# rubengooj/pl-svo

Measured on AMD Instinct MI355X. Metric: sparse-align+pose-opt frames/sec, 640×480, ~200 pts+80 lines; 1/2/4/8 GPU, higher is better.
Workload: dtype f64

## Files before the change

include/plsvo_hip.h:

```cpp
#ifndef PLSVO_HIP_H_
#define PLSVO_HIP_H_

#include <stddef.h>
#include <stdint.h>

#ifdef __cplusplus
extern "C" {
#endif

#define PLSVO_MAX_LEVELS 8
#define PLSVO_PATCH_SIZE 4
#define PLSVO_PATCH_AREA 16

#define PLSVO_OK              0
#define PLSVO_E_INVALID      -1
#define PLSVO_E_NODEVICE     -2
#define PLSVO_E_HIP          -3
#define PLSVO_E_CAPACITY     -4
#define PLSVO_E_STATE        -5
#define PLSVO_E_RCCL         -6

typedef struct plsvo_ctx plsvo_ctx;

typedef struct plsvo_pinhole {
  double fx, fy, cx, cy;
  int32_t width, height;
} plsvo_pinhole;


int plsvo_hip_create(int device_id, void* stream, plsvo_ctx** out);
int plsvo_hip_create_on_stream(int device_id, void* stream, plsvo_ctx** out);
void plsvo_hip_destroy(plsvo_ctx* ctx);
#define PLSVO_OPT_LDLT_FLAVOUR 1
#define PLSVO_OPT_ALIGN_THREADS 2
#define PLSVO_OPT_POSEOPT_THREADS 3
#define PLSVO_OPT_ALIGN_REORDER 4
#define PLSVO_OPT_POSEOPT_REORDER 5
#define PLSVO_OPT_ALIGN_TAIL_SPLIT 6
#define PLSVO_OPT_POSEOPT_REFILL 7
int plsvo_hip_set_option(plsvo_ctx* ctx, int option, int value);
const char* plsvo_hip_last_error(const plsvo_ctx* ctx);
void* plsvo_hip_stream(plsvo_ctx* ctx);
int plsvo_hip_synchronize(plsvo_ctx* ctx);


int plsvo_hip_config_pyramids(plsvo_ctx* ctx, int n_slots, int width, int height, int n_levels);

int plsvo_hip_upload_pyramid(plsvo_ctx* ctx, int slot, int n_levels,
                             const uint8_t* const* level_ptr, const int* width, const int* height,
                             const int* stride_bytes);

int plsvo_hip_build_pyramid(plsvo_ctx* ctx, int slot, const uint8_t* level0, int stride_bytes,
                            int rounding);
int plsvo_hip_build_pyramids_dev(plsvo_ctx* ctx, int first_slot, int n, const void* d_level0,
                                 int stride_bytes, size_t image_pitch_bytes, int rounding);
int plsvo_hip_copy_slots(plsvo_ctx* ctx, int dst_first, int src_first, int n);
int plsvo_hip_download_level(plsvo_ctx* ctx, int slot, int level, uint8_t* out);


typedef struct plsvo_pinhole_radtan {
  plsvo_pinhole cam;
  double d[5];
} plsvo_pinhole_radtan;

#define PLSVO_MAX_RECTIFY_MAPS 8

int plsvo_rectify_map(const plsvo_pinhole_radtan* cam, int16_t* xy, uint16_t* frac);
int plsvo_hip_config_rectify(plsvo_ctx* ctx, const plsvo_pinhole_radtan* cam, int flip_vertical, int* map_id);
int plsvo_hip_rectify_build_pyramid(plsvo_ctx* ctx, int map_id, int slot, const uint8_t* raw, int stride_bytes, int rounding);
int plsvo_hip_rectify_build_pyramids_dev(plsvo_ctx* ctx, int map_id, int first_slot, int n, const void* d_raw,
                                         int stride_bytes, size_t image_pitch_bytes, int rounding);


typedef struct plsvo_corner { int32_t x, y; float score; int32_t level; } plsvo_corner;

typedef struct plsvo_detect_params {
  int32_t cell_size;
  int32_t n_levels;
  int32_t fast_threshold;
  int32_t reserved0;
  double  detection_threshold;
} plsvo_detect_params;

int plsvo_detect_grid(int width, int height, int cell_size, int* cols, int* rows);
int plsvo_detect_cell(int cols, int cell_size, double px_x, double px_y);
int plsvo_hip_detect_fast(plsvo_ctx* ctx, int first_slot, int n, const plsvo_detect_params* params, const uint8_t* occupancy,
                          plsvo_corner* corners, int32_t* counts);
int plsvo_hip_detect_fast_dev(plsvo_ctx* ctx, int first_slot, int n, const plsvo_detect_params* params, const uint8_t* d_occupancy,
                              plsvo_corner* d_corners, int32_t* d_counts);
int plsvo_hip_detect_stages(plsvo_ctx* ctx, int slot, int level, int fast_threshold, uint8_t* score, uint8_t* survives);


typedef struct plsvo_align_in {
  int32_t ref_slot, cur_slot;
  plsvo_pinhole cam;
  int32_t max_level, min_level;
  int32_t n_iter;
  int32_t reserved0;
  double eps;
  double T_cur_from_ref[7];
  int32_t n_pts, n_seg;
  const double* pt_px;
  const double* pt_xyz_ref;
  const double* seg_spx;
  const double* seg_epx;
  const double* seg_len;
  const double* seg_p_ref;
  const double* seg_q_ref;
  const uint8_t* seg_alive_in;
} plsvo_align_in;

typedef struct plsvo_align_out {
  double T_cur_from_ref[7];
  uint64_t n_meas;
  uint64_t n_tracked;
  double H[36];
  double chi2;
  uint8_t* seg_alive_out;
  int32_t iters_per_level[PLSVO_MAX_LEVELS];
  int32_t status;
  int32_t reserved0;
} plsvo_align_out;
// ... 4 lines not shown
  int32_t stop;
  uint64_t n_meas;
  double new_chi2;
  double H[36], Jres[6], x[6];
  double T_after[7];
} plsvo_align_iterlog;

int plsvo_sparse_align(plsvo_ctx* ctx, const plsvo_align_in* in, plsvo_align_out* out);
int plsvo_sparse_align_batch(plsvo_ctx* ctx, int n, const plsvo_align_in* in, plsvo_align_out* out);

int plsvo_align_stage(plsvo_ctx* ctx, int n, const plsvo_align_in* in);
int plsvo_align_run(plsvo_ctx* ctx);
int plsvo_align_fetch(plsvo_ctx* ctx, int n, plsvo_align_out* out);

int plsvo_align_slot_layout(const plsvo_align_in* in, int level, int32_t* seg_code, int32_t* n_slots, int32_t* long_lines,
                            long long* n_patches);

int plsvo_align_set_trace(plsvo_ctx* ctx, int max_records_per_job);
int plsvo_align_fetch_trace(plsvo_ctx* ctx, int job, plsvo_align_iterlog* out, int max_records,
                            int* n_records);

const double* plsvo_align_poses_dev(plsvo_ctx* ctx);
int plsvo_align_copy_poses(plsvo_ctx* ctx, double* d_dst);

int plsvo_align_work(plsvo_ctx* ctx, uint64_t* patch_levels, uint64_t* patch_iters);
int plsvo_align_launch_order(plsvo_ctx* ctx, int n, int32_t* order);
int plsvo_align_tail_frames(plsvo_ctx* ctx, int* tail_frames);
int plsvo_align_work_points(plsvo_ctx* ctx, uint64_t* point_patch_iters);

int plsvo_align_chi2_ties(plsvo_ctx* ctx, uint64_t* iterations, uint64_t* ties, uint64_t* near_ties_without_terms);


typedef struct plsvo_poseopt_in {
  double T_f_w[7];
  double fx;
  double reproj_thresh;
  int32_t n_iter;
  int32_t n_iter_ref;
  int32_t n_pts, n_seg;
  const double* pt_f;
  const double* pt_pos;
  const int32_t* pt_level;
  const double* seg_line;
  const double* seg_spos;
  const double* seg_epos;
  const int32_t* seg_level;
} plsvo_poseopt_in;

typedef struct plsvo_poseopt_out {
  double T_f_w[7];
  double cov[36];
  double estimated_scale, error_init, error_final;
  uint64_t num_obs_pt, num_obs_ls;
  uint8_t* pt_keep;
  uint8_t* seg_keep;
  int32_t iters;
  int32_t iters_ref;
  int32_t status;
  int32_t reserved0;
} plsvo_poseopt_out;

typedef struct plsvo_poseopt_iterlog {
  int32_t phase;
  int32_t iter;
  int32_t accepted;
  int32_t reserved0;
  double new_chi2;
  double A[36], b[6], dT[6];
  double T_after[7];
} plsvo_poseopt_iterlog;

int plsvo_pose_optimize(plsvo_ctx* ctx, const plsvo_poseopt_in* in, plsvo_poseopt_out* out);
int plsvo_pose_optimize_batch(plsvo_ctx* ctx, int n, const plsvo_poseopt_in* in, plsvo_poseopt_out* out);
int plsvo_poseopt_stage(plsvo_ctx* ctx, int n, const plsvo_poseopt_in* in);
int plsvo_poseopt_run(plsvo_ctx* ctx);
int plsvo_poseopt_fetch(plsvo_ctx* ctx, int n, plsvo_poseopt_out* out);
int plsvo_poseopt_set_trace(plsvo_ctx* ctx, int max_records_per_job);
int plsvo_poseopt_fetch_trace(plsvo_ctx* ctx, int job, plsvo_poseopt_iterlog* out, int max_records,
                              int* n_records);
const double* plsvo_poseopt_poses_dev(plsvo_ctx* ctx);
int plsvo_poseopt_copy_poses(plsvo_ctx* ctx, double* d_dst);
int plsvo_poseopt_work(plsvo_ctx* ctx, uint64_t* pt_iters, uint64_t* seg_iters);
int plsvo_poseopt_refill_frames(plsvo_ctx* ctx, int* refill_frames);


typedef struct plsvo_structopt_in {
  int32_t n_frames;
  int32_t n_iter_pts;
  int32_t n_iter_segs;
  int32_t n_pts, n_seg;
  int32_t reserved0;
  const double* frame_T;
  const double* pt_pos;
  const int32_t* pt_obs_off;
  const int32_t* pt_obs_frame;
  const double* pt_obs_f;
  const double* seg_spos;
  const double* seg_epos;
  const int32_t* seg_obs_off;
  const int32_t* seg_obs_frame;
  const double* seg_obs_sf;
  const double* seg_obs_ef;
} plsvo_structopt_in;

typedef struct plsvo_structopt_out {
  double* pt_pos;
  double* seg_spos;
  double* seg_epos;
  int32_t* pt_iters;
  int32_t* seg_iters;
} plsvo_structopt_out;

int plsvo_structure_optimize(plsvo_ctx* ctx, const plsvo_structopt_in* in, plsvo_structopt_out* out);


#define PLSVO_FTR_CORNER  0
#define PLSVO_FTR_EDGELET 1

typedef struct plsvo_match_in {
  plsvo_pinhole cam;
  int32_t n_pyr_levels;
  int32_t align_max_iter;
  int32_t n_frames;
  int32_t n;
  const double* frame_T;
  const int32_t* frame_slot;
  const int32_t* cur_frame;
  const int32_t* ref_frame;
  const double* ref_px;
  const double* ref_f;
  const int32_t* ref_level;
  const uint8_t* ref_type;
  const double* ref_grad;
  const double* pos;
  const double* px_cur;
} plsvo_match_in;

typedef struct plsvo_match_out {
  double* px_cur;
  uint8_t* found;
  int32_t* search_level;
  int32_t* n_iter;
} plsvo_match_out;

int plsvo_match_direct(plsvo_ctx* ctx, const plsvo_match_in* in, plsvo_match_out* out);

typedef struct plsvo_match_warp_out {
  double* A;
  int32_t* search_level;
  uint8_t* warped;
  uint8_t* patch;
  uint8_t* staged;
} plsvo_match_warp_out;

int plsvo_match_warp_patches(plsvo_ctx* ctx, const plsvo_match_in* in, plsvo_match_warp_out* out);

typedef struct plsvo_reproject_in {
  plsvo_pinhole cam;
  int32_t n_frames;
  int32_t n;
  int32_t cell_size;
  int32_t grid_n_cols;
  int32_t boundary;
  int32_t reserved0;
  const double* frame_T;
  const int32_t* frame;
// ... 159 lines not shown
```

pl-svo_amd/abi.py:

```python
import ctypes as C

import numpy as np

MAX_LEVELS = 8
PATCH_AREA = 16

c_double_p = C.POINTER(C.c_double)
c_u8_p = C.POINTER(C.c_uint8)
c_i32_p = C.POINTER(C.c_int32)

OK, E_INVALID, E_NODEVICE, E_HIP, E_CAPACITY, E_STATE, E_RCCL = 0, -1, -2, -3, -4, -5, -6

K_ALIGN_INIT, K_ALIGN_LEVEL, K_POSEOPT, K_HALFSAMPLE, K_STRUCTOPT, K_MATCH, K_SEEDS, K_COUNT = 0, 1, 2, 3, 4, 5, 6, 7
SEED_NOT_VISIBLE, SEED_NO_MATCH, SEED_UPDATED, SEED_CONVERGED, SEED_NAN = 0, 1, 2, 3, 4
FTR_CORNER, FTR_EDGELET = 0, 1


class Pinhole(C.Structure):
    _fields_ = [("fx", C.c_double), ("fy", C.c_double), ("cx", C.c_double), ("cy", C.c_double),
                ("width", C.c_int32), ("height", C.c_int32)]


class PinholeRadtan(C.Structure):
    _fields_ = [("cam", Pinhole), ("d", C.c_double * 5)]
# ... 9 lines not shown


CORNER_DTYPE = np.dtype([("x", np.int32), ("y", np.int32), ("score", np.float32), ("level", np.int32)])


class DetectParams(C.Structure):
    _fields_ = [("cell_size", C.c_int32), ("n_levels", C.c_int32), ("fast_threshold", C.c_int32), ("reserved0", C.c_int32),
                ("detection_threshold", C.c_double)]


def detect_params(cell_size=25, n_levels=3, fast_threshold=20, detection_threshold=20.0):
    return DetectParams(int(cell_size), int(n_levels), int(fast_threshold), 0, float(detection_threshold))


class AlignIn(C.Structure):
    _fields_ = [("ref_slot", C.c_int32), ("cur_slot", C.c_int32), ("cam", Pinhole),
                ("max_level", C.c_int32), ("min_level", C.c_int32), ("n_iter", C.c_int32),
                ("reserved0", C.c_int32), ("eps", C.c_double), ("T_cur_from_ref", C.c_double * 7),
                ("n_pts", C.c_int32), ("n_seg", C.c_int32),
                ("pt_px", c_double_p), ("pt_xyz_ref", c_double_p),
                ("seg_spx", c_double_p), ("seg_epx", c_double_p), ("seg_len", c_double_p),
                ("seg_p_ref", c_double_p), ("seg_q_ref", c_double_p), ("seg_alive_in", c_u8_p)]


class AlignOut(C.Structure):
    _fields_ = [("T_cur_from_ref", C.c_double * 7), ("n_meas", C.c_uint64), ("n_tracked", C.c_uint64),
                ("H", C.c_double * 36), ("chi2", C.c_double), ("seg_alive_out", c_u8_p),
                ("iters_per_level", C.c_int32 * MAX_LEVELS), ("status", C.c_int32), ("reserved0", C.c_int32)]


class AlignIterLog(C.Structure):
    _fields_ = [("level", C.c_int32), ("iter", C.c_int32), ("accepted", C.c_int32), ("stop", C.c_int32),
                ("n_meas", C.c_uint64), ("new_chi2", C.c_double), ("H", C.c_double * 36),
                ("Jres", C.c_double * 6), ("x", C.c_double * 6), ("T_after", C.c_double * 7)]


class PoseOptIn(C.Structure):
    _fields_ = [("T_f_w", C.c_double * 7), ("fx", C.c_double), ("reproj_thresh", C.c_double),
                ("n_iter", C.c_int32), ("n_iter_ref", C.c_int32), ("n_pts", C.c_int32), ("n_seg", C.c_int32),
                ("pt_f", c_double_p), ("pt_pos", c_double_p), ("pt_level", c_i32_p),
                ("seg_line", c_double_p), ("seg_spos", c_double_p), ("seg_epos", c_double_p),
                ("seg_level", c_i32_p)]


class PoseOptOut(C.Structure):
    _fields_ = [("T_f_w", C.c_double * 7), ("cov", C.c_double * 36), ("estimated_scale", C.c_double),
                ("error_init", C.c_double), ("error_final", C.c_double), ("num_obs_pt", C.c_uint64),
                ("num_obs_ls", C.c_uint64), ("pt_keep", c_u8_p), ("seg_keep", c_u8_p), ("iters", C.c_int32),
                ("iters_ref", C.c_int32), ("status", C.c_int32), ("reserved0", C.c_int32)]


class PoseOptIterLog(C.Structure):
    _fields_ = [("phase", C.c_int32), ("iter", C.c_int32), ("accepted", C.c_int32), ("reserved0", C.c_int32),
                ("new_chi2", C.c_double), ("A", C.c_double * 36), ("b", C.c_double * 6), ("dT", C.c_double * 6),
                ("T_after", C.c_double * 7)]


class StructOptIn(C.Structure):
    _fields_ = [("n_frames", C.c_int32), ("n_iter_pts", C.c_int32), ("n_iter_segs", C.c_int32), ("n_pts", C.c_int32),
                ("n_seg", C.c_int32), ("reserved0", C.c_int32), ("frame_T", c_double_p), ("pt_pos", c_double_p),
                ("pt_obs_off", c_i32_p), ("pt_obs_frame", c_i32_p), ("pt_obs_f", c_double_p), ("seg_spos", c_double_p),
                ("seg_epos", c_double_p), ("seg_obs_off", c_i32_p), ("seg_obs_frame", c_i32_p), ("seg_obs_sf", c_double_p),
                ("seg_obs_ef", c_double_p)]


class StructOptOut(C.Structure):
    _fields_ = [("pt_pos", c_double_p), ("seg_spos", c_double_p), ("seg_epos", c_double_p), ("pt_iters", c_i32_p),
                ("seg_iters", c_i32_p)]


class MatchIn(C.Structure):
    _fields_ = [("cam", Pinhole), ("n_pyr_levels", C.c_int32), ("align_max_iter", C.c_int32), ("n_frames", C.c_int32),
                ("n", C.c_int32), ("frame_T", c_double_p), ("frame_slot", c_i32_p), ("cur_frame", c_i32_p),
                ("ref_frame", c_i32_p), ("ref_px", c_double_p), ("ref_f", c_double_p), ("ref_level", c_i32_p),
                ("ref_type", c_u8_p), ("ref_grad", c_double_p), ("pos", c_double_p), ("px_cur", c_double_p)]


class MatchOut(C.Structure):
    _fields_ = [("px_cur", c_double_p), ("found", c_u8_p), ("search_level", c_i32_p), ("n_iter", c_i32_p)]


class MatchWarpOut(C.Structure):
    _fields_ = [("A", c_double_p), ("search_level", c_i32_p), ("warped", c_u8_p), ("patch", c_u8_p), ("staged", c_u8_p)]


class ReprojectIn(C.Structure):
    _fields_ = [("cam", Pinhole), ("n_frames", C.c_int32), ("n", C.c_int32), ("cell_size", C.c_int32), ("grid_n_cols", C.c_int32),
                ("boundary", C.c_int32), ("reserved0", C.c_int32), ("frame_T", c_double_p), ("frame", c_i32_p), ("pos", c_double_p)]


class ReprojectOut(C.Structure):
    _fields_ = [("px", c_double_p), ("cell", c_i32_p)]


class ChainIn(C.Structure):
    _fields_ = [("align", AlignIn), ("T_prev_w", C.c_double * 7), ("T_kf_w", C.c_double * 7), ("kf_slot", C.c_int32),
                ("n_cand_pt", C.c_int32), ("n_cand_seg", C.c_int32), ("reserved0", C.c_int32),
                ("pos", c_double_p), ("ref_px", c_double_p), ("ref_f", c_double_p), ("ref_level", c_i32_p), ("ref_type", c_u8_p),
                ("ref_grad", c_double_p), ("active", c_u8_p)]


class ChainParams(C.Structure):
    _fields_ = [("cam", Pinhole), ("n_pyr_levels", C.c_int32), ("align_max_iter", C.c_int32), ("cell_size", C.c_int32),
                ("cell_rule", C.c_int32), ("max_fts", C.c_int32), ("poseopt_n_iter", C.c_int32), ("cell_order", c_i32_p),
                ("reproj_thresh", C.c_double), ("seg_cell_size", C.c_int32), ("max_fts_segs", C.c_int32), ("seg_cell_order", c_i32_p)]


class ChainOut(C.Structure):
    _fields_ = [("align", AlignOut), ("pose", PoseOptOut), ("n_sel_pt", C.c_int32), ("n_sel_seg", C.c_int32),
                ("found", c_u8_p), ("px", c_double_p), ("search_level", c_i32_p), ("sel_pt", c_i32_p), ("sel_seg", c_i32_p)]


class PoseRecord(C.Structure):
    _fields_ = [("T_f_w", C.c_double * 7), ("n_tracked", C.c_uint64), ("num_obs_pt", C.c_uint64), ("num_obs_ls", C.c_uint64),
                ("error_final", C.c_double), ("status", C.c_int32), ("stream", C.c_int32)]


POSE_RECORD_BYTES = 96
POSE_RECORD_DTYPE = np.dtype([("T_f_w", np.float64, 7), ("n_tracked", np.uint64), ("num_obs_pt", np.uint64), ("num_obs_ls", np.uint64),
                              ("error_final", np.float64), ("status", np.int32), ("stream", np.int32)])
REC_ALIGN, REC_ALIGN_STOP, REC_ALIGN_ERROR, REC_POSEOPT, REC_POSEOPT_EMPTY = 0x01, 0x02, 0x04, 0x08, 0x10

c_float_p = C.POINTER(C.c_float)


class SeedsIn(C.Structure):
    _fields_ = [("cam", Pinhole), ("n_pyr_levels", C.c_int32), ("align_max_iter", C.c_int32), ("max_epi_search_steps", C.c_int32),
                ("edgelet_filtering", C.c_int32), ("edgelet_max_angle", C.c_double), ("px_noise", C.c_double),
                ("convergence_sigma2_thresh", C.c_double), ("n_frames", C.c_int32), ("n_pt", C.c_int32), ("n_seg", C.c_int32),
                ("reserved0", C.c_int32), ("frame_T", c_double_p), ("frame_slot", c_i32_p),
                ("pt_ref_frame", c_i32_p), ("pt_cur_frame", c_i32_p), ("pt_px", c_double_p), ("pt_f", c_double_p), ("pt_level", c_i32_p),
                ("pt_type", c_u8_p), ("pt_grad", c_double_p), ("pt_a", c_float_p), ("pt_b", c_float_p), ("pt_mu", c_float_p),
                ("pt_z_range", c_float_p), ("pt_sigma2", c_float_p),
                ("seg_ref_frame", c_i32_p), ("seg_cur_frame", c_i32_p), ("seg_px", c_double_p), ("seg_f", c_double_p), ("seg_sf", c_double_p),
                ("seg_ef", c_double_p), ("seg_level", c_i32_p), ("seg_a", c_float_p), ("seg_b", c_float_p), ("seg_mu_s", c_float_p),
                ("seg_mu_e", c_float_p), ("seg_z_range_s", c_float_p), ("seg_z_range_e", c_float_p), ("seg_sigma2_s", c_float_p),
                ("seg_sigma2_e", c_float_p)]


class SeedsOut(C.Structure):
    _fields_ = [("pt_status", c_i32_p), ("pt_a", c_float_p), ("pt_b", c_float_p), ("pt_mu", c_float_p), ("pt_sigma2", c_float_p),
                ("pt_xyz_world", c_double_p), ("pt_px_cur", c_double_p), ("pt_depth", c_double_p),
                ("seg_status", c_i32_p), ("seg_a", c_float_p), ("seg_b", c_float_p), ("seg_mu_s", c_float_p), ("seg_mu_e", c_float_p),
                ("seg_sigma2_s", c_float_p), ("seg_sigma2_e", c_float_p), ("seg_xyz_world_s", c_double_p), ("seg_xyz_world_e", c_double_p),
                ("seg_depth_s", c_double_p), ("seg_depth_e", c_double_p)]


def _f64(a, n=None):
    a = np.ascontiguousarray(a, dtype=np.float64)
    if n is not None and a.size != n:
        raise ValueError(f"expected {n} doubles, got {a.size}")
    return a


def _ptr(a, typ):
    return a.ctypes.data_as(typ) if a.size else C.cast(None, typ)


class AlignJob:

    def __init__(self, cam, max_level, min_level, n_iter, eps, T_cur_from_ref, pt_px, pt_xyz_ref,
                 seg_spx, seg_epx, seg_len, seg_p_ref, seg_q_ref, seg_alive_in=None, ref_slot=0, cur_slot=1):
        self.pt_px = _f64(pt_px).reshape(-1, 2)
        n_pts = self.pt_px.shape[0]
        self.pt_xyz_ref = _f64(pt_xyz_ref, 3 * n_pts).reshape(-1, 3)
        self.seg_spx = _f64(seg_spx).reshape(-1, 2)
# ... 308 lines not shown
```

pl-svo_amd/capi.py:

```python
import ctypes as C
import os
import sys

import numpy as np

from . import abi

_HERE = os.path.dirname(os.path.abspath(__file__))
LIB_PATH = os.environ.get("PLSVO_HIP_LIB", os.path.join(_HERE, "libplsvo_hip.so"))

SYMBOLS = [
    "plsvo_hip_create", "plsvo_hip_create_on_stream", "plsvo_hip_set_option", "plsvo_align_slot_layout", "plsvo_hip_destroy", "plsvo_hip_last_error", "plsvo_hip_stream", "plsvo_hip_synchronize",
    "plsvo_hip_config_pyramids", "plsvo_hip_upload_pyramid", "plsvo_hip_build_pyramid", "plsvo_hip_build_pyramids_dev",
    "plsvo_hip_download_level", "plsvo_hip_copy_slots",
    "plsvo_rectify_map", "plsvo_hip_config_rectify", "plsvo_hip_rectify_build_pyramid", "plsvo_hip_rectify_build_pyramids_dev",
    "plsvo_detect_grid", "plsvo_detect_cell", "plsvo_hip_detect_fast", "plsvo_hip_detect_fast_dev", "plsvo_hip_detect_stages",
    "plsvo_sparse_align", "plsvo_sparse_align_batch", "plsvo_align_stage", "plsvo_align_run", "plsvo_align_fetch",
    "plsvo_align_set_trace", "plsvo_align_fetch_trace", "plsvo_align_poses_dev", "plsvo_align_copy_poses", "plsvo_align_work", "plsvo_align_work_points", "plsvo_align_chi2_ties", "plsvo_align_launch_order", "plsvo_align_tail_frames",
    "plsvo_pose_optimize", "plsvo_pose_optimize_batch", "plsvo_poseopt_stage", "plsvo_poseopt_run", "plsvo_poseopt_fetch",
    "plsvo_poseopt_set_trace", "plsvo_poseopt_fetch_trace", "plsvo_poseopt_poses_dev", "plsvo_poseopt_copy_poses", "plsvo_poseopt_work", "plsvo_poseopt_refill_frames",
    "plsvo_structure_optimize", "plsvo_match_direct", "plsvo_match_warp_patches", "plsvo_reproject", "plsvo_trajectory_record", "plsvo_update_seeds",
    "plsvo_chain_stage", "plsvo_chain_run", "plsvo_chain_fetch", "plsvo_frame_step_batch", "plsvo_chain_poses_dev",
    "plsvo_pack_pose_records", "plsvo_fetch_pose_records", "plsvo_gather_poses",
    "plsvo_hip_set_profiling", "plsvo_hip_kernel_time", "plsvo_hip_reset_profiling",
    "plsvo_hip_version", "plsvo_hip_build_flags", "plsvo_hip_device_info",
]


def rectify_map(cam):
    w, h = cam.cam.width, cam.cam.height
    xy = np.zeros((max(h, 0), max(w, 0), 2), dtype=np.int16)
    fr = np.zeros((max(h, 0), max(w, 0)), dtype=np.uint16)
    rc = lib().plsvo_rectify_map(C.byref(cam), xy.ctypes.data_as(C.POINTER(C.c_int16)), fr.ctypes.data_as(C.POINTER(C.c_uint16)))
    if rc != 0:
        raise PlsvoError(rc, "rectify_map: bad camera (non-finite or zero focal length, size outside 1..2046)")
    return xy, fr


def detect_grid(width, height, cell_size):
    cols, rows = C.c_int(0), C.c_int(0)
    rc = lib().plsvo_detect_grid(int(width), int(height), int(cell_size), C.byref(cols), C.byref(rows))
    if rc != 0:
        raise PlsvoError(rc, "detect_grid: width, height and cell_size must be >= 1")
    return cols.value, rows.value


def detect_cell(cols, cell_size, px_x, px_y):
    k = lib().plsvo_detect_cell(int(cols), int(cell_size), float(px_x), float(px_y))
    if k < 0:
        raise PlsvoError(k, "detect_cell: cols and cell_size must be >= 1, the pixel finite and not negative")
    return k


class PlsvoError(RuntimeError):
    def __init__(self, code, msg):
        super().__init__(f"plsvo_hip error {code}: {msg}")
        self.code = code


_lib = None


def lib():
    global _lib
    if _lib is not None:
        return _lib
    if not os.path.exists(LIB_PATH):
        raise ImportError(f"{LIB_PATH} not found: build it with `make -C pl-svo_amd/csrc` "
                          f"(or __graft_entry__.build()); plsvo_hip has no CPU fallback")
    L = C.CDLL(LIB_PATH)
    if hasattr(L, "plsvo_emu_build"):
        sys.stderr.write(f"pl-svo_amd: {LIB_PATH} is a HOST EMULATION build of the kernels (test infrastructure), not the gfx950 library\n")
    ctxp = C.c_void_p
    vp = C.c_void_p
    sig = {
        "plsvo_hip_create": (C.c_int, [C.c_int, vp, C.POINTER(ctxp)]),
        "plsvo_hip_create_on_stream": (C.c_int, [C.c_int, vp, C.POINTER(ctxp)]),
        "plsvo_hip_destroy": (None, [ctxp]),
        "plsvo_hip_set_option": (C.c_int, [ctxp, C.c_int, C.c_int]),
        "plsvo_hip_last_error": (C.c_char_p, [ctxp]),
        "plsvo_hip_stream": (vp, [ctxp]),
        "plsvo_hip_synchronize": (C.c_int, [ctxp]),
        "plsvo_hip_config_pyramids": (C.c_int, [ctxp, C.c_int, C.c_int, C.c_int, C.c_int]),
        "plsvo_hip_upload_pyramid": (C.c_int, [ctxp, C.c_int, C.c_int, C.POINTER(abi.c_u8_p), abi.c_i32_p, abi.c_i32_p, abi.c_i32_p]),
        "plsvo_hip_build_pyramid": (C.c_int, [ctxp, C.c_int, abi.c_u8_p, C.c_int, C.c_int]),
        "plsvo_hip_build_pyramids_dev": (C.c_int, [ctxp, C.c_int, C.c_int, vp, C.c_int, C.c_size_t, C.c_int]),
        "plsvo_hip_download_level": (C.c_int, [ctxp, C.c_int, C.c_int, abi.c_u8_p]),
        "plsvo_hip_copy_slots": (C.c_int, [ctxp, C.c_int, C.c_int, C.c_int]),
        "plsvo_rectify_map": (C.c_int, [C.POINTER(abi.PinholeRadtan), C.POINTER(C.c_int16), C.POINTER(C.c_uint16)]),
        "plsvo_hip_config_rectify": (C.c_int, [ctxp, C.POINTER(abi.PinholeRadtan), C.c_int, C.POINTER(C.c_int)]),
        "plsvo_hip_rectify_build_pyramid": (C.c_int, [ctxp, C.c_int, C.c_int, abi.c_u8_p, C.c_int, C.c_int]),
        "plsvo_hip_rectify_build_pyramids_dev": (C.c_int, [ctxp, C.c_int, C.c_int, C.c_int, vp, C.c_int, C.c_size_t, C.c_int]),
        "plsvo_detect_grid": (C.c_int, [C.c_int, C.c_int, C.c_int, C.POINTER(C.c_int), C.POINTER(C.c_int)]),
        "plsvo_detect_cell": (C.c_int, [C.c_int, C.c_int, C.c_double, C.c_double]),
        "plsvo_hip_detect_fast": (C.c_int, [ctxp, C.c_int, C.c_int, C.POINTER(abi.DetectParams), abi.c_u8_p, C.POINTER(abi.Corner), abi.c_i32_p]),
        "plsvo_hip_detect_fast_dev": (C.c_int, [ctxp, C.c_int, C.c_int, C.POINTER(abi.DetectParams), vp, vp, vp]),
        "plsvo_hip_detect_stages": (C.c_int, [ctxp, C.c_int, C.c_int, C.c_int, abi.c_u8_p, abi.c_u8_p]),
        "plsvo_sparse_align": (C.c_int, [ctxp, C.POINTER(abi.AlignIn), C.POINTER(abi.AlignOut)]),
        "plsvo_sparse_align_batch": (C.c_int, [ctxp, C.c_int, C.POINTER(abi.AlignIn), C.POINTER(abi.AlignOut)]),
        "plsvo_align_stage": (C.c_int, [ctxp, C.c_int, C.POINTER(abi.AlignIn)]),
        "plsvo_align_run": (C.c_int, [ctxp]),
        "plsvo_align_fetch": (C.c_int, [ctxp, C.c_int, C.POINTER(abi.AlignOut)]),
        "plsvo_align_set_trace": (C.c_int, [ctxp, C.c_int]),
        "plsvo_align_fetch_trace": (C.c_int, [ctxp, C.c_int, C.POINTER(abi.AlignIterLog), C.c_int, C.POINTER(C.c_int)]),
        "plsvo_align_poses_dev": (vp, [ctxp]),
        "plsvo_align_copy_poses": (C.c_int, [ctxp, vp]),
        "plsvo_poseopt_copy_poses": (C.c_int, [ctxp, vp]),
        "plsvo_align_work": (C.c_int, [ctxp, C.POINTER(C.c_uint64), C.POINTER(C.c_uint64)]),
        "plsvo_align_chi2_ties": (C.c_int, [ctxp, C.POINTER(C.c_uint64), C.POINTER(C.c_uint64), C.POINTER(C.c_uint64)]),
        "plsvo_align_work_points": (C.c_int, [ctxp, C.POINTER(C.c_uint64)]),
        "plsvo_align_launch_order": (C.c_int, [ctxp, C.c_int, C.POINTER(C.c_int32)]),
        "plsvo_align_tail_frames": (C.c_int, [ctxp, C.POINTER(C.c_int)]),
        "plsvo_poseopt_refill_frames": (C.c_int, [ctxp, C.POINTER(C.c_int)]),
        "plsvo_pose_optimize": (C.c_int, [ctxp, C.POINTER(abi.PoseOptIn), C.POINTER(abi.PoseOptOut)]),
        "plsvo_pose_optimize_batch": (C.c_int, [ctxp, C.c_int, C.POINTER(abi.PoseOptIn), C.POINTER(abi.PoseOptOut)]),
        "plsvo_poseopt_stage": (C.c_int, [ctxp, C.c_int, C.POINTER(abi.PoseOptIn)]),
        "plsvo_poseopt_run": (C.c_int, [ctxp]),
        "plsvo_poseopt_fetch": (C.c_int, [ctxp, C.c_int, C.POINTER(abi.PoseOptOut)]),
        "plsvo_poseopt_set_trace": (C.c_int, [ctxp, C.c_int]),
        "plsvo_poseopt_fetch_trace": (C.c_int, [ctxp, C.c_int, C.POINTER(abi.PoseOptIterLog), C.c_int, C.POINTER(C.c_int)]),
        "plsvo_poseopt_poses_dev": (vp, [ctxp]),
        "plsvo_poseopt_work": (C.c_int, [ctxp, C.POINTER(C.c_uint64), C.POINTER(C.c_uint64)]),
        "plsvo_structure_optimize": (C.c_int, [ctxp, C.POINTER(abi.StructOptIn), C.POINTER(abi.StructOptOut)]),
        "plsvo_match_direct": (C.c_int, [ctxp, C.POINTER(abi.MatchIn), C.POINTER(abi.MatchOut)]),
        "plsvo_match_warp_patches": (C.c_int, [ctxp, C.POINTER(abi.MatchIn), C.POINTER(abi.MatchWarpOut)]),
        "plsvo_reproject": (C.c_int, [ctxp, C.POINTER(abi.ReprojectIn), C.POINTER(abi.ReprojectOut)]),
        "plsvo_update_seeds": (C.c_int, [ctxp, C.POINTER(abi.SeedsIn), C.POINTER(abi.SeedsOut)]),
        "plsvo_trajectory_record": (C.c_int, [abi.c_double_p, abi.c_double_p, abi.c_double_p]),
        "plsvo_chain_stage": (C.c_int, [ctxp, C.c_int, C.POINTER(abi.ChainIn), C.POINTER(abi.ChainParams)]),
        "plsvo_chain_run": (C.c_int, [ctxp]),
        "plsvo_chain_fetch": (C.c_int, [ctxp, C.c_int, C.POINTER(abi.ChainOut)]),
        "plsvo_frame_step_batch": (C.c_int, [ctxp, C.c_int, C.POINTER(abi.ChainIn), C.POINTER(abi.ChainParams), C.POINTER(abi.ChainOut)]),
        "plsvo_chain_poses_dev": (vp, [ctxp]),
        "plsvo_align_slot_layout": (C.c_int, [C.POINTER(abi.AlignIn), C.c_int, C.POINTER(C.c_int32), C.POINTER(C.c_int32), C.POINTER(C.c_int32),
                                              C.POINTER(C.c_longlong)]),
        "plsvo_pack_pose_records": (C.c_int, [ctxp, vp, C.POINTER(C.c_int)]),
        "plsvo_fetch_pose_records": (C.c_int, [ctxp, C.c_int, C.POINTER(abi.PoseRecord)]),
        "plsvo_gather_poses": (C.c_int, [ctxp, vp, vp, C.c_int, vp]),
        "plsvo_hip_set_profiling": (C.c_int, [ctxp, C.c_int]),
        "plsvo_hip_kernel_time": (C.c_int, [ctxp, C.c_int, C.POINTER(C.c_double), C.POINTER(C.c_int64)]),
        "plsvo_hip_reset_profiling": (C.c_int, [ctxp]),
        "plsvo_hip_version": (C.c_char_p, []),
        "plsvo_hip_build_flags": (C.c_char_p, []),
        "plsvo_hip_device_info": (C.c_int, [ctxp, C.c_char_p, C.c_int, C.POINTER(C.c_int), C.POINTER(C.c_size_t)]),
    }
    for name, (res, args) in sig.items():
        if "PLSVO_HIP_LIB" in os.environ and not hasattr(L, name):
            continue
        f = getattr(L, name)
        f.restype = res
        f.argtypes = args
    _lib = L
    return L


class Context:

    def __init__(self, device=0, stream=None):
        self.L = lib()
        h = C.c_void_p()
        if stream is None:
            rc = self.L.plsvo_hip_create(int(device), None, C.byref(h))
        else:
            rc = self.L.plsvo_hip_create_on_stream(int(device), C.c_void_p(int(stream)), C.byref(h))
        if rc != 0:
            raise PlsvoError(rc, (self.L.plsvo_hip_last_error(None) or b"").decode())
        self.h = h
        self._keep = None

    def set_ldlt_flavour(self, flavour):
        self._chk(self.L.plsvo_hip_set_option(self.h, 1, int(flavour)))

    def set_launch_shapes(self, align_threads=None, poseopt_threads=None):
        if align_threads is not None:
            self._chk(self.L.plsvo_hip_set_option(self.h, 2, int(align_threads)))
        if poseopt_threads is not None:
            self._chk(self.L.plsvo_hip_set_option(self.h, 3, int(poseopt_threads)))

    def set_launch_order_refresh(self, align=None, poseopt=None):
        if align is not None:
            self._chk(self.L.plsvo_hip_set_option(self.h, 4, 1 if align else 0))
        if poseopt is not None:
            self._chk(self.L.plsvo_hip_set_option(self.h, 5, 1 if poseopt else 0))

    def set_align_tail_split(self, on):
        self._chk(self.L.plsvo_hip_set_option(self.h, 6, 1 if on else 0))

    def set_poseopt_refill(self, on):
        self._chk(self.L.plsvo_hip_set_option(self.h, 7, 1 if on else 0))

    def close(self):
        if getattr(self, "h", None):
            self.L.plsvo_hip_destroy(self.h)
            self.h = None

    def __del__(self):
        try:
            self.close()
        except Exception:
            pass

    def _chk(self, rc):
        if rc != 0:
            raise PlsvoError(rc, (self.L.plsvo_hip_last_error(self.h) or b"").decode())

    def device_info(self):
        name = C.create_string_buffer(256)
        cu = C.c_int(0)
        mem = C.c_size_t(0)
        self._chk(self.L.plsvo_hip_device_info(self.h, name, 256, C.byref(cu), C.byref(mem)))
        return name.value.decode(), cu.value, mem.value

    def stream(self):
        return self.L.plsvo_hip_stream(self.h)

    def synchronize(self):
        self._chk(self.L.plsvo_hip_synchronize(self.h))

    def set_profiling(self, on):
        self._chk(self.L.plsvo_hip_set_profiling(self.h, 1 if on else 0))

    def reset_profiling(self):
        self._chk(self.L.plsvo_hip_reset_profiling(self.h))

    def kernel_time(self, k):
        ms = C.c_double(0)
        n = C.c_int64(0)
        self._chk(self.L.plsvo_hip_kernel_time(self.h, k, C.byref(ms), C.byref(n)))
        return ms.value, n.value

    def config_pyramids(self, n_slots, width, height, n_levels):
        self._chk(self.L.plsvo_hip_config_pyramids(self.h, n_slots, width, height, n_levels))
        self.n_levels = n_levels
        self.width, self.height = width, height

    def upload_pyramid(self, slot, levels):
        keep = [np.ascontiguousarray(l, dtype=np.uint8) for l in levels]
        n = len(keep)
        ptrs = (abi.c_u8_p * n)(*[l.ctypes.data_as(abi.c_u8_p) for l in keep])
        w = (C.c_int32 * n)(*[l.shape[1] for l in keep])
        h = (C.c_int32 * n)(*[l.shape[0] for l in keep])
        s = (C.c_int32 * n)(*[l.strides[0] for l in keep])
        self._chk(self.L.plsvo_hip_upload_pyramid(self.h, slot, n, ptrs, w, h, s))

    def build_pyramid(self, slot, img0, rounding=0):
        img0 = np.ascontiguousarray(img0, dtype=np.uint8)
        self._chk(self.L.plsvo_hip_build_pyramid(self.h, slot, img0.ctypes.data_as(abi.c_u8_p), img0.strides[0], rounding))

    def build_pyramids_dev(self, first_slot, n, d_ptr, stride_bytes, image_pitch_bytes, rounding=0):
        self._chk(self.L.plsvo_hip_build_pyramids_dev(self.h, first_slot, n, C.c_void_p(d_ptr), stride_bytes,
                                                      image_pitch_bytes, rounding))

    def download_level(self, slot, level):
        w, h = self.width >> level, self.height >> level
        out = np.empty((h, w), dtype=np.uint8)
        self._chk(self.L.plsvo_hip_download_level(self.h, slot, level, out.ctypes.data_as(abi.c_u8_p)))
        return out

    def copy_slots(self, dst_first, src_first, n):
        self._chk(self.L.plsvo_hip_copy_slots(self.h, int(dst_first), int(src_first), int(n)))

    def download_pyramid(self, slot):
        return [self.download_level(slot, l) for l in range(self.n_levels)]

    def config_rectify(self, cam, flip_vertical=False):
        mid = C.c_int(-1)
        self._chk(self.L.plsvo_hip_config_rectify(self.h, C.byref(cam), 1 if flip_vertical else 0, C.byref(mid)))
        return mid.value

    def rectify_build_pyramid(self, map_id, slot, raw, rounding=0):
        raw = np.asarray(raw, dtype=np.uint8)
        if raw.ndim != 2 or raw.strides[1] != 1:
            raw = np.ascontiguousarray(raw)
# ... 3 lines not shown
    def rectify_build_pyramids_dev(self, map_id, first_slot, n, d_ptr, stride_bytes, image_pitch_bytes, rounding=0):
        self._chk(self.L.plsvo_hip_rectify_build_pyramids_dev(self.h, int(map_id), int(first_slot), int(n), C.c_void_p(d_ptr),
                                                              int(stride_bytes), int(image_pitch_bytes), int(rounding)))

    def detect_fast(self, first_slot, n, cell_size=25, n_levels=3, fast_threshold=20, detection_threshold=20.0, occupancy=None):
        cols, rows = detect_grid(self.width, self.height, cell_size)
        cells = cols * rows
        pr = abi.detect_params(cell_size, n_levels, fast_threshold, detection_threshold)
        occ = None
        if occupancy is not None:
            occ = np.ascontiguousarray(np.asarray(occupancy).reshape(int(n), cells) != 0, dtype=np.uint8)
        out = np.zeros((max(int(n), 1), cells), dtype=abi.CORNER_DTYPE)
        counts = np.zeros(max(int(n), 1), dtype=np.int32)
        self._chk(self.L.plsvo_hip_detect_fast(self.h, int(first_slot), int(n), C.byref(pr), None if occ is None else occ.ctypes.data_as(abi.c_u8_p),
                                               out.ctypes.data_as(C.POINTER(abi.Corner)), counts.ctypes.data_as(abi.c_i32_p)))
        return [out[i, :counts[i]].copy() for i in range(int(n))]

    def detect_fast_dev(self, first_slot, n, d_corners, d_counts, cell_size=25, n_levels=3, fast_threshold=20, detection_threshold=20.0,
                        d_occupancy=None):
        pr = abi.detect_params(cell_size, n_levels, fast_threshold, detection_threshold)
        self._chk(self.L.plsvo_hip_detect_fast_dev(self.h, int(first_slot), int(n), C.byref(pr), C.c_void_p(d_occupancy), C.c_void_p(d_corners),
                                                   C.c_void_p(d_counts)))

    def detect_stages(self, slot, level, fast_threshold=20):
        w, h = self.width >> level, self.height >> level
        score = np.zeros((max(h, 0), max(w, 0)), dtype=np.uint8)
        surv = np.zeros_like(score)
        self._chk(self.L.plsvo_hip_detect_stages(self.h, int(slot), int(level), int(fast_threshold), score.ctypes.data_as(abi.c_u8_p),
                                                 surv.ctypes.data_as(abi.c_u8_p)))
        return score, surv

    def align_set_trace(self, max_records):
        self._chk(self.L.plsvo_align_set_trace(self.h, max_records))
        self._align_trace = max_records

    def align_stage(self, jobs):
        arr = (abi.AlignIn * len(jobs))(*[j.c for j in jobs])
        self._chk(self.L.plsvo_align_stage(self.h, len(jobs), arr))
        self._align_jobs = jobs

    def align_run(self):
        self._chk(self.L.plsvo_align_run(self.h))

    def align_fetch(self):
        jobs = self._align_jobs
        n = len(jobs)
        outs = (abi.AlignOut * n)()
        alive = [np.ones(max(j.n_seg, 1), dtype=np.uint8) for j in jobs]
        for o, a in zip(outs, alive):
            o.seg_alive_out = a.ctypes.data_as(abi.c_u8_p)
        self._chk(self.L.plsvo_align_fetch(self.h, n, outs))
        return [abi.AlignResult(o, a[:j.n_seg].copy()) for o, a, j in zip(outs, alive, jobs)]

    def align_fetch_trace(self, job):
        cap = getattr(self, "_align_trace", 0)
        log = (abi.AlignIterLog * max(cap, 1))()
        n = C.c_int(0)
        self._chk(self.L.plsvo_align_fetch_trace(self.h, job, log, cap, C.byref(n)))
        return abi.align_log_to_dicts(log, n.value)

    def sparse_align_batch(self, jobs):
        self.align_stage(jobs)
        self.align_run()
        return self.align_fetch()

    def sparse_align(self, job):
        return self.sparse_align_batch([job])[0]

    def align_work(self):
        a = C.c_uint64(0)
        b = C.c_uint64(0)
        self._chk(self.L.plsvo_align_work(self.h, C.byref(a), C.byref(b)))
        return a.value, b.value

    def align_work_points(self):
        a = C.c_uint64(0)
        self._chk(self.L.plsvo_align_work_points(self.h, C.byref(a)))
        return a.value

    def align_launch_order(self, n):
        out = np.zeros(n, dtype=np.int32)
        self._chk(self.L.plsvo_align_launch_order(self.h, n, out.ctypes.data_as(C.POINTER(C.c_int32))))
        return out

    def poseopt_refill_frames(self):
        n = C.c_int(0)
        self._chk(self.L.plsvo_poseopt_refill_frames(self.h, C.byref(n)))
        return n.value

    def align_tail_frames(self):
        n = C.c_int(0)
        self._chk(self.L.plsvo_align_tail_frames(self.h, C.byref(n)))
        return n.value

    def align_chi2_ties(self):
        a = C.c_uint64(0)
        b = C.c_uint64(0)
        c = C.c_uint64(0)
        self._chk(self.L.plsvo_align_chi2_ties(self.h, C.byref(a), C.byref(b), C.byref(c)))
        return a.value, b.value, c.value

    def align_poses_dev(self):
        return self.L.plsvo_align_poses_dev(self.h)

    def align_copy_poses(self, d_dst):
        self._chk(self.L.plsvo_align_copy_poses(self.h, C.c_void_p(d_dst)))

    def poseopt_copy_poses(self, d_dst):
        self._chk(self.L.plsvo_poseopt_copy_poses(self.h, C.c_void_p(d_dst)))

    def poseopt_set_trace(self, max_records):
        self._chk(self.L.plsvo_poseopt_set_trace(self.h, max_records))
        self._pose_trace = max_records

    def poseopt_stage(self, jobs):
        arr = (abi.PoseOptIn * len(jobs))(*[j.c for j in jobs])
        self._chk(self.L.plsvo_poseopt_stage(self.h, len(jobs), arr))
        self._pose_jobs = jobs

    def poseopt_run(self):
        self._chk(self.L.plsvo_poseopt_run(self.h))

    def poseopt_fetch(self):
        jobs = self._pose_jobs
        n = len(jobs)
        outs = (abi.PoseOptOut * n)()
        pk = [np.ones(max(j.n_pts, 1), dtype=np.uint8) for j in jobs]
        sk = [np.ones(max(j.n_seg, 1), dtype=np.uint8) for j in jobs]
        for o, a, b in zip(outs, pk, sk):
            o.pt_keep = a.ctypes.data_as(abi.c_u8_p)
            o.seg_keep = b.ctypes.data_as(abi.c_u8_p)
        self._chk(self.L.plsvo_poseopt_fetch(self.h, n, outs))
        return [abi.PoseOptResult(o, a[:j.n_pts].copy(), b[:j.n_seg].copy()) for o, a, b, j in zip(outs, pk, sk, jobs)]

    def poseopt_fetch_trace(self, job):
        cap = getattr(self, "_pose_trace", 0)
        log = (abi.PoseOptIterLog * max(cap, 1))()
        n = C.c_int(0)
        self._chk(self.L.plsvo_poseopt_fetch_trace(self.h, job, log, cap, C.byref(n)))
        return abi.poseopt_log_to_dicts(log, n.value)

    def pose_optimize_batch(self, jobs):
        self.poseopt_stage(jobs)
        self.poseopt_run()
        return self.poseopt_fetch()

    def pose_optimize(self, job):
        return self.pose_optimize_batch([job])[0]

    def poseopt_work(self):
        a = C.c_uint64(0)
        b = C.c_uint64(0)
        self._chk(self.L.plsvo_poseopt_work(self.h, C.byref(a), C.byref(b)))
        return a.value, b.value

    def poseopt_poses_dev(self):
        return self.L.plsvo_poseopt_poses_dev(self.h)

    def chain_stage(self, jobs, cam, n_pyr_levels=3, align_max_iter=10, cell_size=30, cell_rule=False, max_fts=120, cell_order=None,
                    reproj_thresh=2.0, poseopt_n_iter=10, seg_cell_size=0, max_fts_segs=100, seg_cell_order=None):
        n = len(jobs)
        arr = (abi.ChainIn * n)(*[j.c for j in jobs])
        pr = abi.ChainParams()
        pr.cam = cam if isinstance(cam, abi.Pinhole) else abi.Pinhole(*cam)
        pr.n_pyr_levels, pr.align_max_iter, pr.cell_size, pr.cell_rule = int(n_pyr_levels), int(align_max_iter), int(cell_size), int(bool(cell_rule))
        pr.max_fts, pr.poseopt_n_iter, pr.reproj_thresh = int(max_fts), int(poseopt_n_iter), float(reproj_thresh)
# ... 103 lines not shown
```

pl-svo_amd/csrc/plsvo_capi.hip:

```cpp
#include <hip/hip_runtime.h>
#include <dlfcn.h>
#include <rccl/rccl.h>

#include <algorithm>
#include <chrono>
#include <cmath>
#include <cstdio>
#include <cstdlib>
#include <cstring>
#include <string>
#include <vector>

#include "../../include/plsvo_hip.h"
#include "plsvo_dev.hpp"
#include "plsvo_math.hpp"
#include "poseopt_refill.hpp"

namespace plsvo_hip {
size_t align_level_lds_bytes(int threads, int cap, int scap, int chi_lds_pts);
hipError_t launch_align_reorder(const int* work_key, int n, int* order_out, int shift, hipStream_t stream);
hipError_t launch_align_levels(const AlignBatchDev& b, int cap, int scap, int level_hi, int level_lo, int do_init, int threads, size_t lds,
                               hipStream_t stream);
hipError_t launch_pose_opt(const PoseBatchDev& b, double* d_poses, int threads, hipStream_t stream);
hipError_t launch_structopt(const StructBatchDev& s, hipStream_t stream);
hipError_t launch_match_direct(const MatchBatchDev& b, hipStream_t stream);
hipError_t launch_match_warp_patches(const MatchBatchDev& b, hipStream_t stream);
hipError_t launch_reproject(const ReprojBatchDev& b, hipStream_t stream);
hipError_t launch_update_seeds(const SeedsBatchDev& b, hipStream_t stream);
hipError_t launch_halfsample(const uint8_t* src, size_t src_pitch, int in_w, int in_h, int in_stride, uint8_t* dst,
                             size_t dst_pitch, int n_slots, int rounding, hipStream_t stream);
hipError_t launch_copy_level0(const uint8_t* src, size_t src_pitch, int w, int h, int stride, uint8_t* dst, size_t dst_pitch,
                              int n_slots, hipStream_t stream);
hipError_t launch_chain_pose(const ChainBatchDev& b, hipStream_t stream);
hipError_t launch_pack_pose_records(const AlignStateDev* ast, const PoseStateDev* pst, int n, plsvo_pose_record* dst, hipStream_t stream);
hipError_t launch_chain_active(const ChainBatchDev& b, hipStream_t stream);
hipError_t launch_chain_select(const ChainBatchDev& b, hipStream_t stream);
hipError_t launch_tile_level(const uint8_t* src, size_t src_pitch, int w, int h, uint8_t* dst, size_t dst_pitch, int n_slots, hipStream_t stream);
hipError_t launch_rectify(const uint8_t* raw, size_t raw_pitch, int stride, int flip, const uint32_t* map, int w, int h, uint8_t* dst,
                          size_t dst_pitch, int n_slots, hipStream_t stream);
hipError_t launch_detect_fast(const DetectLaunch& a, int n_slots, hipStream_t stream);
hipError_t launch_detect_stages(const DetectLaunch& a, hipStream_t stream);
hipError_t launch_detect_compact(unsigned long long* keys, int n_cells, plsvo_corner* corners, int32_t* counts, int n_slots, hipStream_t stream);
}

using namespace plsvo_hip;

static thread_local std::string g_create_error;

namespace {

struct DevBuf {
  void* p = nullptr;
  size_t cap = 0;
  hipError_t ensure(size_t bytes) {
    if (bytes <= cap) return hipSuccess;
    if (p) { hipError_t e = hipFree(p); p = nullptr; cap = 0; if (e != hipSuccess) return e; }
    size_t want = std::max(bytes, (size_t)256);
    hipError_t e = hipMalloc(&p, want);
    if (e == hipSuccess) cap = want;
    return e;
  }
  void release() { if (p) (void)hipFree(p); p = nullptr; cap = 0; }
  template <typename T> T* as() const { return reinterpret_cast<T*>(p); }
};

struct EventPair { hipEvent_t a, b; };

struct Blob {
  std::vector<uint8_t> host;
  template <typename T> size_t add(const std::vector<T>& v) {
    const size_t off = (host.size() + 255) & ~(size_t)255;
    host.resize(off + std::max(v.size() * sizeof(T), (size_t)16));
    if (!v.empty()) memcpy(host.data() + off, v.data(), v.size() * sizeof(T));
    return off;
  }
};

}

struct plsvo_ctx {
  int device = 0;
  hipStream_t stream = nullptr;
  bool own_stream = false;
  std::string err;
  int cu_count = 0;
  size_t lds_per_block = 65536;
  int env_align_threads = 0, env_align_lds_pad = 0, env_poseopt_threads = 0;
  bool env_align_per_level = false, env_align_no_lpt = false, env_host_timing = false;
  int ldlt_flavour = 320;

  DevBuf pyr_tiled;
  DevBuf pyr_slab;
  PyrDesc pyr{};
  DevBuf pyr_upload;
  struct RectifyMap { DevBuf map; int w = 0, h = 0; bool identity = false, flip = false; };
  RectifyMap rect[PLSVO_MAX_RECTIFY_MAPS];
  int rect_n = 0;
  DevBuf det_keys, det_occ, det_corners, det_counts, det_stage;

  int a_n = 0;
  bool a_staged = false;
  std::vector<AlignJobDev> a_jobs;
  std::vector<int> a_nseg_off;
  int a_total_seg = 0;
  int a_gmax = -1, a_gmin = 99;
  int a_cap[PLSVO_MAX_LEVELS]{};
  int a_scap = 4;
  int a_trace_cap = 0;
  DevBuf a_d_state, a_d_alive;
  DevBuf a_d_pxyz, a_d_puv, a_d_cref, a_d_chi, a_d_log, a_d_poses;
  size_t a_patch_total = 0;
  int a_seg_align = 32;
  DevBuf a_d_workkey;
  DevBuf a_d_order[2];
  int a_order_next = 0;
  bool env_align_no_reorder = false;
  const int* a_stage_order = nullptr;
  bool a_one_shot = false, p_one_shot = false;
  int env_align_reorder_min = 0;
  bool opt_align_tail_split = true;
  int env_align_tail_min = 0, env_align_tail_k = 0, env_align_tail_frames = 0;
  DevBuf a_d_tailflag;
  DevBuf a_d_alive_tail;
  DevBuf a_d_xbuf;
  unsigned int x_launch = 0;
  bool env_align_no_pair = false;
  AlignBatchDev a_b{};

  int p_n = 0;
  bool p_staged = false;
  std::vector<PoseJobDev> p_jobs;
  int p_total_pt = 0, p_total_seg = 0;
  int p_trace_cap = 0;
  DevBuf p_d_state, p_d_ptkeep, p_d_segkeep;
  DevBuf p_d_s32, p_d_s64, p_d_log, p_d_poses;
  PoseBatchDev p_b{};
  DevBuf p_d_workkey, p_d_order[2];
  int p_order_next = 0, p_key_shift = 0;
  bool env_poseopt_no_reorder = false;
  int env_poseopt_reorder_min = 0;
  bool opt_poseopt_refill = true;
  int env_poseopt_refill_min = 0, env_poseopt_refill_waves = 0;
  bool p_any_ref = false;
  int p_refill_frames = 0;
  DevBuf p_d_carry, p_d_refill_next;

  bool ch_staged = false;
  int ch_n = 0, ch_ncand = 0, ch_npt_cap = 0, ch_nseg_cap = 0;
  std::vector<ChainJobDev> ch_jobs;
  DevBuf ch_d_blob, ch_d_work, ch_d_po;
  ChainBatchDev ch_b{};
  MatchBatchDev ch_match{};
  ReprojBatchDev ch_reproj{};
  PoseBatchDev ch_pose{};
  DevBuf ch_d_state, ch_d_ptkeep, ch_d_segkeep, ch_d_s32, ch_d_s64, ch_d_poses;
  DevBuf rec_d;
  unsigned long long run_seq = 0, a_run_seq = 0, p_run_seq = 0, ch_run_seq = 0;

  DevBuf s_d_in, s_d_out;

  DevBuf a_d_blob, p_d_blob;
  void* pinned[2] = { nullptr, nullptr };
  size_t pinned_cap[2] = { 0, 0 };
  hipEvent_t pinned_done[2] = { nullptr, nullptr };
  int pinned_next = 0;
  void* pyr_pinned[2] = { nullptr, nullptr };
  size_t pyr_pinned_cap[2] = { 0, 0 };
  hipEvent_t pyr_pinned_done[2] = { nullptr, nullptr };
  int pyr_pinned_next = 0;
  std::vector<uint8_t> tiled_stale;
  int tiled_stale_count = 0;
  void* dl_pinned = nullptr;
  size_t dl_pinned_cap = 0;

  bool profiling = false;
  std::vector<EventPair> ev[PLSVO_K_COUNT];
  std::vector<EventPair> ev_pool;
  double ev_ms[PLSVO_K_COUNT]{};
  int64_t ev_launches[PLSVO_K_COUNT]{};
};

#define CTX_CHECK(ctx) do { if (!(ctx)) return PLSVO_E_INVALID; } while (0)
#define HIP_TRY(ctx, expr)                                                                      \
  do {                                                                                          \
    hipError_t e__ = (expr);                                                                    \
    if (e__ != hipSuccess) {                                                                    \
      (ctx)->err = std::string(#expr) + ": " + hipGetErrorString(e__);                          \
      return PLSVO_E_HIP;                                                                       \
    }                                                                                           \
  } while (0)
static int fail(plsvo_ctx* ctx, int code, const std::string& msg) { ctx->err = msg; return code; }

static void prof_begin(plsvo_ctx* c, int k, EventPair* ep) {
  if (!c->profiling) return;
  if (!c->ev_pool.empty()) { *ep = c->ev_pool.back(); c->ev_pool.pop_back(); }
  else { (void)hipEventCreate(&ep->a); (void)hipEventCreate(&ep->b); }
  (void)hipEventRecord(ep->a, c->stream);
  (void)k;
}
static void prof_end(plsvo_ctx* c, int k, EventPair* ep) {
  if (!c->profiling) return;
  (void)hipEventRecord(ep->b, c->stream);
  c->ev[k].push_back(*ep);
}
static void prof_collect(plsvo_ctx* c) {
  for (int k = 0; k < PLSVO_K_COUNT; ++k) {
    for (auto& ep : c->ev[k]) {
      float ms = 0.f;
      if (hipEventSynchronize(ep.b) == hipSuccess && hipEventElapsedTime(&ms, ep.a, ep.b) == hipSuccess) {
        c->ev_ms[k] += (double)ms; c->ev_launches[k] += 1;
      }
      c->ev_pool.push_back(ep);
    }
    c->ev[k].clear();
  }
}

extern "C" const char* plsvo_hip_version(void) { return "plsvo_hip 0.1 (gfx950)"; }

static int create_ctx(int device_id, void* stream, bool use_given_stream, plsvo_ctx** out);
static bool env_flag(const char* name) { const char* s = getenv(name); return s && *s && strcmp(s, "0") != 0; }
extern "C" int plsvo_hip_create(int device_id, void* stream, plsvo_ctx** out) { return create_ctx(device_id, stream, stream != nullptr, out); }
extern "C" int plsvo_hip_create_on_stream(int device_id, void* stream, plsvo_ctx** out) { return create_ctx(device_id, stream, true, out); }

static int create_ctx(int device_id, void* stream, bool use_given_stream, plsvo_ctx** out) {
  if (!out) return PLSVO_E_INVALID;
  *out = nullptr;
  int n = 0;
  hipError_t e = hipGetDeviceCount(&n);
  if (e != hipSuccess || n <= 0) {
    g_create_error = std::string("no HIP device available (") + (e != hipSuccess ? hipGetErrorString(e) : "count=0") +
                     "); plsvo_hip has no CPU fallback";
    return PLSVO_E_NODEVICE;
  }
  if (device_id < 0 || device_id >= n) { g_create_error = "device_id out of range"; return PLSVO_E_INVALID; }
  if ((e = hipSetDevice(device_id)) != hipSuccess) { g_create_error = hipGetErrorString(e); return PLSVO_E_HIP; }
  plsvo_ctx* c = new plsvo_ctx();
  c->device = device_id;
  hipDeviceProp_t prop;
  if (hipGetDeviceProperties(&prop, device_id) == hipSuccess) {
    c->cu_count = prop.multiProcessorCount;
    c->lds_per_block = prop.sharedMemPerBlock;
    int optin = 0;
    if (hipDeviceGetAttribute(&optin, hipDeviceAttributeMaxSharedMemoryPerBlock, device_id) == hipSuccess && optin > 0)
      c->lds_per_block = std::max(c->lds_per_block, (size_t)optin);
  }
  if (use_given_stream) { c->stream = reinterpret_cast<hipStream_t>(stream); c->own_stream = false; }
  else {
    if ((e = hipStreamCreateWithFlags(&c->stream, hipStreamNonBlocking)) != hipSuccess) {
      g_create_error = hipGetErrorString(e); delete c; return PLSVO_E_HIP;
    }
    c->own_stream = true;
  }
  if (const char* s = getenv("PLSVO_LDS_LIMIT")) c->lds_per_block = (size_t)atol(s);
  if (const char* s = getenv("PLSVO_ALIGN_THREADS")) { const int v = atoi(s); if (v == 64 || v == 128 || v == 256 || v == 512) c->env_align_threads = v; }
  if (const char* s = getenv("PLSVO_ALIGN_LDS_PAD")) c->env_align_lds_pad = std::max(0, atoi(s));
  if (const char* s = getenv("PLSVO_POSEOPT_THREADS")) { const int v = atoi(s); if (v == 16 || v == 64 || v == 256 || v == 512) c->env_poseopt_threads = v; }
  if (const char* s = getenv("PLSVO_ALIGN_PER_LEVEL")) c->env_align_per_level = atoi(s) != 0;
  c->env_align_no_lpt = env_flag("PLSVO_ALIGN_NO_LPT");
  c->env_align_no_pair = env_flag("PLSVO_ALIGN_NO_PAIR");
  c->env_align_no_reorder = env_flag("PLSVO_ALIGN_NO_REORDER");
  if (const char* s = getenv("PLSVO_ALIGN_REORDER_MIN")) c->env_align_reorder_min = atoi(s);
  if (const char* s = getenv("PLSVO_ALIGN_TAIL_SPLIT")) c->opt_align_tail_split = atoi(s) != 0;
  if (const char* s = getenv("PLSVO_ALIGN_TAIL_MIN")) c->env_align_tail_min = atoi(s);
  if (const char* s = getenv("PLSVO_ALIGN_TAIL_K")) c->env_align_tail_k = atoi(s);
  if (const char* s = getenv("PLSVO_ALIGN_TAIL_FRAMES")) c->env_align_tail_frames = atoi(s);
  c->env_poseopt_no_reorder = env_flag("PLSVO_POSEOPT_NO_REORDER");
  if (const char* s = getenv("PLSVO_POSEOPT_REORDER_MIN")) c->env_poseopt_reorder_min = atoi(s);
  if (const char* s = getenv("PLSVO_POSEOPT_REFILL")) c->opt_poseopt_refill = atoi(s) != 0;
  if (const char* s = getenv("PLSVO_POSEOPT_REFILL_MIN")) c->env_poseopt_refill_min = atoi(s);
  if (const char* s = getenv("PLSVO_POSEOPT_REFILL_WAVES")) c->env_poseopt_refill_waves = atoi(s);
  c->env_host_timing = getenv("PLSVO_HOST_TIMING") != nullptr;
  *out = c;
  return PLSVO_OK;
}

extern "C" void plsvo_hip_destroy(plsvo_ctx* c) {
  if (!c) return;
  (void)hipSetDevice(c->device);
  (void)hipStreamSynchronize(c->stream);
  prof_collect(c);
  for (auto& ep : c->ev_pool) { (void)hipEventDestroy(ep.a); (void)hipEventDestroy(ep.b); }
  c->a_d_tailflag.release(); c->a_d_alive_tail.release(); c->a_d_xbuf.release(); c->a_d_order[0].release(); c->a_d_order[1].release(); c->a_d_workkey.release(); c->p_d_workkey.release(); c->p_d_order[0].release(); c->p_d_order[1].release();
  c->p_d_carry.release(); c->p_d_refill_next.release();
  DevBuf* bufs[] = { &c->pyr_slab, &c->pyr_tiled, &c->pyr_upload, &c->a_d_blob, &c->a_d_state, &c->a_d_alive, &c->a_d_pxyz, &c->a_d_puv, &c->a_d_cref,
                     &c->a_d_chi, &c->a_d_log, &c->a_d_poses, &c->p_d_blob, &c->p_d_state, &c->p_d_ptkeep, &c->p_d_segkeep, &c->p_d_s32, &c->p_d_s64,
                     &c->p_d_log, &c->p_d_poses, &c->s_d_in, &c->s_d_out, &c->ch_d_blob, &c->ch_d_work, &c->ch_d_po, &c->ch_d_state,
                     &c->ch_d_ptkeep, &c->ch_d_segkeep, &c->ch_d_s32, &c->ch_d_s64, &c->ch_d_poses, &c->rec_d };
  for (DevBuf* b : bufs) b->release();
  for (auto& r : c->rect) r.map.release();
  c->det_keys.release(); c->det_occ.release(); c->det_corners.release(); c->det_counts.release(); c->det_stage.release();
  for (int k = 0; k < 2; ++k) { if (c->pinned[k]) (void)hipHostFree(c->pinned[k]); if (c->pinned_done[k]) (void)hipEventDestroy(c->pinned_done[k]); }
  for (int k = 0; k < 2; ++k) { if (c->pyr_pinned[k]) (void)hipHostFree(c->pyr_pinned[k]); if (c->pyr_pinned_done[k]) (void)hipEventDestroy(c->pyr_pinned_done[k]); }
  if (c->dl_pinned) (void)hipHostFree(c->dl_pinned);
  if (c->own_stream) (void)hipStreamDestroy(c->stream);
  delete c;
}

extern "C" int plsvo_hip_set_option(plsvo_ctx* c, int option, int value) {
  CTX_CHECK(c);
  if (option == PLSVO_OPT_LDLT_FLAVOUR) {
    if (value != 320 && value != 330) return fail(c, PLSVO_E_INVALID, "set_option: the LDLT flavour is 320 (Eigen 3.1 ... 3.2.1) or 330 (Eigen 3.2.2 and later)");
    c->ldlt_flavour = value;
    c->a_staged = false; c->p_staged = false;
    return PLSVO_OK;
  }
  if (option == PLSVO_OPT_ALIGN_THREADS) {
    if (value != 0 && value != 64 && value != 128 && value != 256 && value != 512) return fail(c, PLSVO_E_INVALID, "set_option: alignment launch shape is 0 (automatic), 64, 128, 256 or 512 threads per frame");
    c->env_align_threads = value;
    return PLSVO_OK;
  }
  if (option == PLSVO_OPT_POSEOPT_THREADS) {
    if (value != 0 && value != 16 && value != 64 && value != 256 && value != 512) return fail(c, PLSVO_E_INVALID, "set_option: pose-optimiser launch shape is 0 (automatic), 16 (a 16-lane row per frame, four frames per wave), 64, 256 or 512 threads per frame");
    c->env_poseopt_threads = value;
    return PLSVO_OK;
  }
  if (option == PLSVO_OPT_ALIGN_REORDER || option == PLSVO_OPT_POSEOPT_REORDER) {
    if (value != 0 && value != 1) return fail(c, PLSVO_E_INVALID, "set_option: the launch-order refresh is 0 (keep the stage order) or 1 (refresh from the last launch's measured work)");
    if (option == PLSVO_OPT_ALIGN_REORDER) {
      c->env_align_no_reorder = value == 0;
      if (value == 0 && c->a_staged && c->a_d_blob.p) c->a_b.order = c->a_stage_order;
    } else {
      c->env_poseopt_no_reorder = value == 0;
    }
    return PLSVO_OK;
  }
  if (option == PLSVO_OPT_ALIGN_TAIL_SPLIT) {
    if (value != 0 && value != 1) return fail(c, PLSVO_E_INVALID, "set_option: the alignment's tail split is 0 (one workgroup per frame throughout) or 1 (the frames that start last run as a coarse and a fine part)");
    c->opt_align_tail_split = value != 0;
    return PLSVO_OK;
  }
  if (option == PLSVO_OPT_POSEOPT_REFILL) {
    if (value != 0 && value != 1) return fail(c, PLSVO_E_INVALID, "set_option: the pose optimiser's row refill is 0 (four frames of a wave in lock step) or 1 (rows take their next frame from a queue)");
    c->opt_poseopt_refill = value != 0;
    return PLSVO_OK;
  }
  return fail(c, PLSVO_E_INVALID, "set_option: unknown option");
}

extern "C" const char* plsvo_hip_last_error(const plsvo_ctx* c) { return c ? c->err.c_str() : g_create_error.c_str(); }
extern "C" void* plsvo_hip_stream(plsvo_ctx* c) { return c ? reinterpret_cast<void*>(c->stream) : nullptr; }
extern "C" int plsvo_hip_synchronize(plsvo_ctx* c) { CTX_CHECK(c); HIP_TRY(c, hipStreamSynchronize(c->stream)); return PLSVO_OK; }

extern "C" int plsvo_hip_device_info(plsvo_ctx* c, char* name, int name_len, int* cu_count, size_t* hbm_bytes) {
  CTX_CHECK(c);
  hipDeviceProp_t prop;
  HIP_TRY(c, hipGetDeviceProperties(&prop, c->device));
  if (name && name_len > 0) { snprintf(name, (size_t)name_len, "%s (%s)", prop.name, prop.gcnArchName); }
  if (cu_count) *cu_count = prop.multiProcessorCount;
  if (hbm_bytes) *hbm_bytes = prop.totalGlobalMem;
  return PLSVO_OK;
}

extern "C" int plsvo_hip_config_pyramids(plsvo_ctx* c, int n_slots, int width, int height, int n_levels) {
  CTX_CHECK(c);
  if (n_slots <= 0 || width <= 0 || height <= 0 || n_levels <= 0 || n_levels > PLSVO_MAX_LEVELS) return fail(c, PLSVO_E_INVALID, "config_pyramids: bad arguments");
  HIP_TRY(c, hipSetDevice(c->device));
  PyrDesc d{};
  size_t off = 0;
  for (int l = 0; l < n_levels; ++l) {
    d.w[l] = width >> l; d.h[l] = height >> l;
    if (d.w[l] <= 0 || d.h[l] <= 0) return fail(c, PLSVO_E_INVALID, "config_pyramids: too many levels for this image size");
    d.off[l] = pyr_level_offset(width, height, l);
    off = (size_t)pyr_level_offset(width, height, l + 1);
  }
  d.slot_bytes = off; d.n_slots = n_slots; d.n_levels = n_levels;
  d.tslot_bytes = pyr_tiled_level_offset(width, height, n_levels);
  HIP_TRY(c, hipStreamSynchronize(c->stream));
  HIP_TRY(c, c->pyr_slab.ensure((size_t)n_slots * off + 256));
  HIP_TRY(c, hipMemsetAsync(c->pyr_slab.p, 0, (size_t)n_slots * off + 256, c->stream));
  HIP_TRY(c, c->pyr_tiled.ensure((size_t)n_slots * d.tslot_bytes + 256));
  HIP_TRY(c, hipMemsetAsync(c->pyr_tiled.p, 0, (size_t)n_slots * d.tslot_bytes + 256, c->stream));
  d.base = c->pyr_slab.as<uint8_t>();
  d.tbase = c->pyr_tiled.as<uint8_t>();
  c->pyr = d;
  c->tiled_stale.assign((size_t)n_slots, 0); c->tiled_stale_count = 0;
  c->a_staged = false;
  c->ch_staged = false;
  return PLSVO_OK;
}

static int check_slot(plsvo_ctx* c, int slot) {
  if (!c->pyr.base) return fail(c, PLSVO_E_STATE, "pyramids not configured");
  if (slot < 0 || slot >= c->pyr.n_slots) return fail(c, PLSVO_E_CAPACITY, "pyramid slot out of range");
  return PLSVO_OK;
}

static int retile(plsvo_ctx* c, int first_slot, int n, int n_levels) {
  const uint8_t* src = c->pyr_slab.as<uint8_t>() + (size_t)first_slot * c->pyr.slot_bytes;
  uint8_t* dst = c->pyr_tiled.as<uint8_t>() + (size_t)first_slot * c->pyr.tslot_bytes;
  for (int l = 0; l < n_levels; ++l)
    HIP_TRY(c, launch_tile_level(src + c->pyr.off[l], c->pyr.slot_bytes, c->pyr.w[l], c->pyr.h[l],
                                 dst + pyr_tiled_level_offset(c->pyr.w[0], c->pyr.h[0], l), c->pyr.tslot_bytes, n, c->stream));
  return PLSVO_OK;
}

static void mark_tiled_fresh(plsvo_ctx* c, int first, int n) {
  if (c->tiled_stale_count == 0) return;
  for (int s = first; s < first + n && s < (int)c->tiled_stale.size(); ++s)
    if (c->tiled_stale[(size_t)s]) { c->tiled_stale[(size_t)s] = 0; --c->tiled_stale_count; }
}
static int retile_stale(plsvo_ctx* c, const std::vector<int>& slots) {
  if (c->tiled_stale_count == 0) return PLSVO_OK;
  for (int sl : slots) {
    if (sl < 0 || sl >= (int)c->tiled_stale.size() || !c->tiled_stale[(size_t)sl]) continue;
    int rc = retile(c, sl, 1, c->pyr.n_levels); if (rc) return rc;
    c->tiled_stale[(size_t)sl] = 0; --c->tiled_stale_count;
    if (c->tiled_stale_count == 0) break;
  }
  return PLSVO_OK;
}

extern "C" int plsvo_hip_upload_pyramid(plsvo_ctx* c, int slot, int n_levels, const uint8_t* const* level_ptr, const int* width,
                                        const int* height, const int* stride_bytes) {
  CTX_CHECK(c);
  int rc = check_slot(c, slot); if (rc) return rc;
  if (!level_ptr || !width || !height || !stride_bytes || n_levels <= 0 || n_levels > c->pyr.n_levels) return fail(c, PLSVO_E_INVALID, "upload_pyramid: bad arguments");
// ... 945 lines not shown
    for (int k = 0; k < 7; ++k) J.T0[k] = a.T_f_w[k];
    J.fx = a.fx; J.reproj_thresh = a.reproj_thresh; J.n_iter = a.n_iter; J.n_iter_ref = a.n_iter_ref; J.ldlt_flavour = c->ldlt_flavour; J.reserved0 = 0;
    J.pt_off = (int)plev.size(); J.n_pts = a.n_pts; J.seg_off = (int)slev.size(); J.n_seg = a.n_seg;
    f.insert(f.end(), a.pt_f, a.pt_f + 3 * (size_t)a.n_pts);
    pos.insert(pos.end(), a.pt_pos, a.pt_pos + 3 * (size_t)a.n_pts);
    plev.insert(plev.end(), a.pt_level, a.pt_level + (size_t)a.n_pts);
    line.insert(line.end(), a.seg_line, a.seg_line + 3 * (size_t)a.n_seg);
    spos.insert(spos.end(), a.seg_spos, a.seg_spos + 3 * (size_t)a.n_seg);
    epos.insert(epos.end(), a.seg_epos, a.seg_epos + 3 * (size_t)a.n_seg);
    slev.insert(slev.end(), a.seg_level, a.seg_level + (size_t)a.n_seg);
    for (int i = 0; i < a.n_pts; ++i) if (a.pt_level[i] < 0 || a.pt_level[i] > 30) return fail(c, PLSVO_E_INVALID, "poseopt_stage: feature level out of range");
    for (int i = 0; i < a.n_seg; ++i) if (a.seg_level[i] < 0 || a.seg_level[i] > 30) return fail(c, PLSVO_E_INVALID, "poseopt_stage: feature level out of range");
  }
  int rc;
  Blob blob;
  const size_t o_jobs = blob.add(jobs), o_f = blob.add(f), o_pos = blob.add(pos), o_plev = blob.add(plev), o_line = blob.add(line),
               o_spos = blob.add(spos), o_epos = blob.add(epos), o_slev = blob.add(slev);
  if ((rc = upload_blob(c, c->p_d_blob, blob))) return rc;
  const size_t npt = plev.size(), nsg = slev.size(), nft = std::max(npt + nsg, (size_t)1);
  HIP_TRY(c, c->p_d_ptkeep.ensure(std::max(npt, (size_t)1)));
  HIP_TRY(c, c->p_d_segkeep.ensure(std::max(nsg, (size_t)1)));
  HIP_TRY(c, c->p_d_s32.ensure(nft * sizeof(float)));
  HIP_TRY(c, c->p_d_s64.ensure(nft * 5 * sizeof(double)));
  HIP_TRY(c, c->p_d_state.ensure((size_t)n * sizeof(PoseStateDev)));
  HIP_TRY(c, c->p_d_poses.ensure((size_t)n * 7 * sizeof(double)));
  if (c->p_trace_cap > 0) HIP_TRY(c, c->p_d_log.ensure((size_t)n * c->p_trace_cap * sizeof(plsvo_poseopt_iterlog)));
  PoseBatchDev& b = c->p_b;
  uint8_t* const base = c->p_d_blob.as<uint8_t>();
  b.jobs = reinterpret_cast<const PoseJobDev*>(base + o_jobs); b.state = c->p_d_state.as<PoseStateDev>();
  b.pt_f = reinterpret_cast<const double*>(base + o_f); b.pt_pos = reinterpret_cast<const double*>(base + o_pos);
  b.pt_level = reinterpret_cast<const int*>(base + o_plev);
  b.seg_line = reinterpret_cast<const double*>(base + o_line); b.seg_spos = reinterpret_cast<const double*>(base + o_spos);
  b.seg_epos = reinterpret_cast<const double*>(base + o_epos); b.seg_level = reinterpret_cast<const int*>(base + o_slev);
  b.pt_keep = c->p_d_ptkeep.as<uint8_t>(); b.seg_keep = c->p_d_segkeep.as<uint8_t>();
  b.scratch_f32 = c->p_d_s32.as<float>(); b.scratch_f64 = c->p_d_s64.as<double>();
  b.log = c->p_trace_cap > 0 ? c->p_d_log.as<plsvo_poseopt_iterlog>() : nullptr;
  b.log_cap = c->p_trace_cap; b.n_jobs = n;
  b.order = nullptr; b.work_key = nullptr;
  {
    long key_max = 1;
    for (int j = 0; j < n; ++j) key_max = std::max(key_max, (long)(jobs[j].n_pts + jobs[j].n_seg) * (long)(std::max(jobs[j].n_iter, 0) + std::max(jobs[j].n_iter_ref, 0)));
    c->p_key_shift = 0;
    while ((key_max >> c->p_key_shift) > 1023) ++c->p_key_shift;
  }
  c->p_any_ref = false;
  for (int j = 0; j < n; ++j) c->p_any_ref = c->p_any_ref || jobs[j].n_iter_ref > 0;
  c->p_jobs.swap(jobs);
  c->p_n = n; c->p_total_pt = (int)npt; c->p_total_seg = (int)nsg;
  c->p_staged = true; c->p_run_seq = 0;
  return PLSVO_OK;
}

extern "C" int plsvo_poseopt_run(plsvo_ctx* c) {
  CTX_CHECK(c);
  RoctxRange range("pose_optimizer");
  if (!c->p_staged) return fail(c, PLSVO_E_STATE, "poseopt_run: no staged batch");
  HIP_TRY(c, hipSetDevice(c->device));
  const int cus = c->cu_count > 0 ? c->cu_count : 256;
  const long feats = (long)c->p_total_pt + (long)c->p_total_seg;
  int threads = c->p_n <= 2 * cus ? 256 : (feats <= 580l * c->p_n ? 16 : 64);
  if (c->env_poseopt_threads) threads = c->env_poseopt_threads;
  const bool reorder = threads != 256 && !c->env_poseopt_no_reorder && !c->p_one_shot &&
                       c->p_n > (c->env_poseopt_reorder_min > 0 ? c->env_poseopt_reorder_min - 1 : (threads == 16 ? 4 : 8) * cus);
  c->p_b.work_key = nullptr;
  if (reorder) {
    if (c->p_d_workkey.cap < (size_t)c->p_n * sizeof(int)) {
      HIP_TRY(c, c->p_d_workkey.ensure((size_t)c->p_n * sizeof(int)));
      HIP_TRY(c, hipMemsetAsync(c->p_d_workkey.p, 0, c->p_d_workkey.cap, c->stream));
    }
    c->p_b.work_key = c->p_d_workkey.as<int>();
  } else c->p_b.order = nullptr;
  const int resident_wgs = cus * 512 / 64;
  const int refill_min = c->env_poseopt_refill_min > 0 ? c->env_poseopt_refill_min : 2 * 4 * resident_wgs + 1;
  const bool refill = c->opt_poseopt_refill && threads == 16 && !c->p_b.log && !c->p_any_ref && pose_opt_refill_built() && c->p_n >= refill_min;
  c->p_refill_frames = 0;
  EventPair ep{}; prof_begin(c, PLSVO_K_POSEOPT, &ep);
  if (refill) {
    const int wgs = (c->p_n + 3) / 4;
    const int gn_grid = std::max(1, std::min(wgs, c->env_poseopt_refill_waves > 0 ? c->env_poseopt_refill_waves : resident_wgs));
    HIP_TRY(c, c->p_d_carry.ensure((size_t)c->p_n * sizeof(PoseRefillCarry)));
    HIP_TRY(c, c->p_d_refill_next.ensure(16));
    HIP_TRY(c, hipMemsetAsync(c->p_d_refill_next.p, 0, 16, c->stream));
    const PoseRefillDev q{ c->p_d_carry.as<PoseRefillCarry>(), c->p_d_refill_next.as<int>() };
    HIP_TRY(c, launch_pose_opt_refill(c->p_b, q, c->p_d_poses.as<double>(), gn_grid, c->stream));
    c->p_refill_frames = c->p_n;
  } else {
    HIP_TRY(c, launch_pose_opt(c->p_b, c->p_d_poses.as<double>(), threads, c->stream));
  }
  c->p_run_seq = ++c->run_seq;
  prof_end(c, PLSVO_K_POSEOPT, &ep);
  if (reorder) {
    DevBuf& ob = c->p_d_order[c->p_order_next];
    HIP_TRY(c, ob.ensure((size_t)c->p_n * sizeof(int)));
    HIP_TRY(c, launch_align_reorder(c->p_b.work_key, c->p_n, ob.as<int>(), c->p_key_shift, c->stream));
    c->p_b.order = ob.as<int>();
    c->p_order_next ^= 1;
  }
  return PLSVO_OK;
}

extern "C" int plsvo_poseopt_fetch(plsvo_ctx* c, int n, plsvo_poseopt_out* out) {
  CTX_CHECK(c);
  if (!c->p_staged) return fail(c, PLSVO_E_STATE, "poseopt_fetch: no staged batch");
  if (n != c->p_n || !out) return fail(c, PLSVO_E_INVALID, "poseopt_fetch: n does not match the staged batch");
  HIP_TRY(c, hipSetDevice(c->device));
  std::vector<uint8_t> big;
  const size_t rb[3] = { (size_t)n * sizeof(PoseStateDev), (size_t)std::max(c->p_total_pt, 0), (size_t)std::max(c->p_total_seg, 0) };
  const void* const rs[3] = { c->p_d_state.p, c->p_d_ptkeep.p, c->p_d_segkeep.p };
  const uint8_t* rh[3] = { nullptr, nullptr, nullptr };
  { const int rc_d = download_ranges(c, 3, rs, rb, big, rh); if (rc_d) return rc_d; }
  const PoseStateDev* const st = reinterpret_cast<const PoseStateDev*>(rh[0]);
  const uint8_t* const pk = rh[1]; const uint8_t* const sk = rh[2];
  for (int j = 0; j < n; ++j) {
    const PoseStateDev& s = st[(size_t)j];
    const PoseJobDev& J = c->p_jobs[(size_t)j];
    plsvo_poseopt_out& o = out[j];
    uint8_t* pko = o.pt_keep; uint8_t* sko = o.seg_keep;
    memset(&o, 0, sizeof(o));
    o.pt_keep = pko; o.seg_keep = sko;
    for (int k = 0; k < 7; ++k) o.T_f_w[k] = s.T[k];
    for (int k = 0; k < 36; ++k) o.cov[k] = s.cov[k];
    o.estimated_scale = s.estimated_scale; o.error_init = s.error_init; o.error_final = s.error_final;
    o.num_obs_pt = s.num_obs_pt; o.num_obs_ls = s.num_obs_ls;
    o.iters = s.iters; o.iters_ref = s.iters_ref; o.status = s.status;
    if (pko && J.n_pts > 0) memcpy(pko, pk + J.pt_off, (size_t)J.n_pts);
    if (sko && J.n_seg > 0) memcpy(sko, sk + J.seg_off, (size_t)J.n_seg);
  }
  return PLSVO_OK;
}

extern "C" int plsvo_poseopt_refill_frames(plsvo_ctx* c, int* refill_frames) {
  CTX_CHECK(c);
  if (!refill_frames) return fail(c, PLSVO_E_INVALID, "poseopt_refill_frames: NULL output");
  *refill_frames = c->p_refill_frames;
  return PLSVO_OK;
}

extern "C" int plsvo_pose_optimize_batch(plsvo_ctx* c, int n, const plsvo_poseopt_in* in, plsvo_poseopt_out* out) {
  int rc = plsvo_poseopt_stage(c, n, in); if (rc) return rc;
  c->p_one_shot = true;
  rc = plsvo_poseopt_run(c);
  c->p_one_shot = false;
  if (rc) return rc;
  return plsvo_poseopt_fetch(c, n, out);
}
extern "C" int plsvo_pose_optimize(plsvo_ctx* c, const plsvo_poseopt_in* in, plsvo_poseopt_out* out) {
  return plsvo_pose_optimize_batch(c, 1, in, out);
}

extern "C" int plsvo_poseopt_set_trace(plsvo_ctx* c, int max_records_per_job) {
  CTX_CHECK(c);
  if (max_records_per_job < 0) return fail(c, PLSVO_E_INVALID, "set_trace: negative capacity");
  c->p_trace_cap = max_records_per_job;
  c->p_staged = false;
  return PLSVO_OK;
}

extern "C" int plsvo_poseopt_fetch_trace(plsvo_ctx* c, int job, plsvo_poseopt_iterlog* out, int max_records, int* n_records) {
  CTX_CHECK(c);
  if (!c->p_staged || c->p_trace_cap <= 0) return fail(c, PLSVO_E_STATE, "fetch_trace: tracing not enabled for the staged batch");
  if (job < 0 || job >= c->p_n || !out || !n_records) return fail(c, PLSVO_E_INVALID, "fetch_trace: bad arguments");
  HIP_TRY(c, hipSetDevice(c->device));
  PoseStateDev s;
  HIP_TRY(c, hipMemcpyAsync(&s, c->p_d_state.as<PoseStateDev>() + job, sizeof(s), hipMemcpyDeviceToHost, c->stream));
  HIP_TRY(c, hipStreamSynchronize(c->stream));
  const int nrec = std::min(std::min(s.log_count, c->p_trace_cap), max_records);
  if (nrec > 0) {
    HIP_TRY(c, hipMemcpyAsync(out, c->p_d_log.as<plsvo_poseopt_iterlog>() + (size_t)job * c->p_trace_cap, (size_t)nrec * sizeof(plsvo_poseopt_iterlog),
                              hipMemcpyDeviceToHost, c->stream));
    HIP_TRY(c, hipStreamSynchronize(c->stream));
  }
  *n_records = nrec;
  return PLSVO_OK;
}

extern "C" const double* plsvo_poseopt_poses_dev(plsvo_ctx* c) { return (c && c->p_staged) ? c->p_d_poses.as<double>() : nullptr; }

extern "C" int plsvo_poseopt_copy_poses(plsvo_ctx* c, double* d_dst) {
  CTX_CHECK(c);
  if (!c->p_staged || !d_dst) return fail(c, PLSVO_E_STATE, "poseopt_copy_poses: no staged batch / null destination");
  HIP_TRY(c, hipSetDevice(c->device));
  HIP_TRY(c, hipMemcpyAsync(d_dst, c->p_d_poses.p, (size_t)c->p_n * 7 * sizeof(double), hipMemcpyDeviceToDevice, c->stream));
  return PLSVO_OK;
}

extern "C" int plsvo_poseopt_work(plsvo_ctx* c, uint64_t* pt_iters, uint64_t* seg_iters) {
  CTX_CHECK(c);
  if (!c->p_staged) return fail(c, PLSVO_E_STATE, "poseopt_work: no staged batch");
  HIP_TRY(c, hipSetDevice(c->device));
  std::vector<PoseStateDev> st((size_t)c->p_n);
  HIP_TRY(c, hipMemcpyAsync(st.data(), c->p_d_state.p, (size_t)c->p_n * sizeof(PoseStateDev), hipMemcpyDeviceToHost, c->stream));
  HIP_TRY(c, hipStreamSynchronize(c->stream));
  uint64_t a = 0, b2 = 0;
  for (auto& s : st) { a += s.pt_iters; b2 += s.seg_iters; }
  if (pt_iters) *pt_iters = a;
  if (seg_iters) *seg_iters = b2;
  return PLSVO_OK;
}

extern "C" int plsvo_structure_optimize(plsvo_ctx* c, const plsvo_structopt_in* in, plsvo_structopt_out* out) {
  CTX_CHECK(c);
  if (!in || !out || in->n_pts < 0 || in->n_seg < 0 || in->n_frames < 0 || in->n_iter_pts < 0 || in->n_iter_segs < 0)
    return fail(c, PLSVO_E_INVALID, "structure_optimize: bad arguments");
  if ((in->n_pts > 0 && (!in->pt_pos || !in->pt_obs_off)) || (in->n_seg > 0 && (!in->seg_spos || !in->seg_epos || !in->seg_obs_off)))
    return fail(c, PLSVO_E_INVALID, "structure_optimize: null landmark array");
  if (in->n_pts + in->n_seg == 0) return PLSVO_OK;
  HIP_TRY(c, hipSetDevice(c->device));
  const int np = in->n_pts, ns = in->n_seg;
  const int npo = np > 0 ? in->pt_obs_off[np] : 0, nso = ns > 0 ? in->seg_obs_off[ns] : 0;
  if (npo < 0 || nso < 0 || (npo > 0 && (!in->pt_obs_frame || !in->pt_obs_f)) || (nso > 0 && (!in->seg_obs_frame || !in->seg_obs_sf || !in->seg_obs_ef)) ||
      ((npo > 0 || nso > 0) && (!in->frame_T || in->n_frames <= 0)))
    return fail(c, PLSVO_E_INVALID, "structure_optimize: bad observation tables");
  for (int i = 0; i < npo; ++i) if (in->pt_obs_frame[i] < 0 || in->pt_obs_frame[i] >= in->n_frames) return fail(c, PLSVO_E_INVALID, "structure_optimize: frame index out of range");
  for (int i = 0; i < nso; ++i) if (in->seg_obs_frame[i] < 0 || in->seg_obs_frame[i] >= in->n_frames) return fail(c, PLSVO_E_INVALID, "structure_optimize: frame index out of range");
  std::vector<double> d;
  auto putd = [&](const double* p, size_t n) { const size_t o = d.size(); if (n) d.insert(d.end(), p, p + n); return o; };
  const size_t o_T = putd(in->frame_T, (size_t)in->n_frames * 7), o_pp = putd(in->pt_pos, (size_t)np * 3), o_pf = putd(in->pt_obs_f, (size_t)npo * 3);
// ... 251 lines not shown
  HIP_TRY(c, c->ch_d_work.ensure(w.off + 256));
  Carver p;
  const size_t p_jobs = p.take<PoseJobDev>((size_t)n), p_ptf = p.take<double>((size_t)npt_total * 3), p_ptpos = p.take<double>((size_t)npt_total * 3),
               p_ptlev = p.take<int>((size_t)npt_total), p_line = p.take<double>((size_t)nseg_total * 3), p_spos = p.take<double>((size_t)nseg_total * 3),
               p_epos = p.take<double>((size_t)nseg_total * 3), p_slev = p.take<int>((size_t)nseg_total);
  HIP_TRY(c, c->ch_d_po.ensure(p.off + 256));
  const size_t nft = std::max((size_t)npt_total + (size_t)nseg_total, (size_t)1);
  HIP_TRY(c, c->ch_d_ptkeep.ensure(std::max((size_t)npt_total, (size_t)1)));
  HIP_TRY(c, c->ch_d_segkeep.ensure(std::max((size_t)nseg_total, (size_t)1)));
  HIP_TRY(c, c->ch_d_s32.ensure(nft * sizeof(float)));
  HIP_TRY(c, c->ch_d_s64.ensure(nft * 5 * sizeof(double)));
  HIP_TRY(c, c->ch_d_state.ensure((size_t)n * sizeof(PoseStateDev)));
  HIP_TRY(c, c->ch_d_poses.ensure((size_t)n * 7 * sizeof(double)));
  uint8_t* const B = c->ch_d_blob.as<uint8_t>();
  uint8_t* const Wk = c->ch_d_work.as<uint8_t>();
  uint8_t* const Po = c->ch_d_po.as<uint8_t>();
  ChainBatchDev& b = c->ch_b;
  b = ChainBatchDev{};
  b.jobs = reinterpret_cast<const ChainJobDev*>(B + o_jobs); b.n_jobs = n; b.n_cand = (int)NC;
  b.align_poses = c->a_d_poses.as<double>();
  b.frame_T = reinterpret_cast<double*>(Wk + w_frameT); b.frame_slot = reinterpret_cast<int*>(Wk + w_fslot);
  b.cand_job = reinterpret_cast<const int*>(B + o_cjob); b.pos = reinterpret_cast<const double*>(B + o_pos);
  b.active_in = any_active ? B + o_active : nullptr;
  b.cell = reinterpret_cast<const int*>(Wk + w_cell); b.active = Wk + w_act;
  b.m_px = reinterpret_cast<const double*>(Wk + w_mpx); b.found = Wk + w_found; b.search_level = reinterpret_cast<const int*>(Wk + w_slevel);
  b.fx = pr->cam.fx; b.fy = pr->cam.fy; b.cx = pr->cam.cx; b.cy = pr->cam.cy;
  b.n_cells = n_cells; b.cell_rule = pr->cell_rule ? 1 : 0; b.max_fts = pr->max_fts;
  b.cell_order = pr->cell_rule ? reinterpret_cast<const int*>(B + o_order) : nullptr;
  b.proj_px = reinterpret_cast<const double*>(Wk + w_px);
  b.seg_cell_size = seg_grid ? pr->seg_cell_size : 0; b.seg_n_cols = seg_n_cols; b.seg_n_cells = seg_n_cells; b.max_fts_segs = pr->max_fts_segs;
  b.seg_cell_order = seg_grid ? reinterpret_cast<const int*>(B + o_sorder) : nullptr;
  b.po_jobs = reinterpret_cast<PoseJobDev*>(Po + p_jobs);
  b.pt_f = reinterpret_cast<double*>(Po + p_ptf); b.pt_pos = reinterpret_cast<double*>(Po + p_ptpos); b.pt_level = reinterpret_cast<int*>(Po + p_ptlev);
  b.seg_line = reinterpret_cast<double*>(Po + p_line); b.seg_spos = reinterpret_cast<double*>(Po + p_spos); b.seg_epos = reinterpret_cast<double*>(Po + p_epos);
  b.seg_level = reinterpret_cast<int*>(Po + p_slev);
  b.sel_pt = reinterpret_cast<int*>(Wk + w_selpt); b.sel_seg = reinterpret_cast<int*>(Wk + w_selseg); b.n_sel = reinterpret_cast<int*>(Wk + w_nsel);
  b.reproj_thresh = pr->reproj_thresh; b.po_n_iter = pr->poseopt_n_iter; b.ldlt_flavour = c->ldlt_flavour;
  ReprojBatchDev& r = c->ch_reproj;
  r = ReprojBatchDev{};
  r.fx = pr->cam.fx; r.fy = pr->cam.fy; r.cx = pr->cam.cx; r.cy = pr->cam.cy; r.cam_width = pr->cam.width; r.cam_height = pr->cam.height;
  r.n = (int)NC; r.cell_size = pr->cell_size; r.grid_n_cols = grid_n_cols; r.boundary = 8;
  r.frame_T = b.frame_T; r.frame = reinterpret_cast<const int*>(B + o_fcur); r.pos = b.pos;
  r.px = reinterpret_cast<double*>(Wk + w_px); r.cell = reinterpret_cast<int*>(Wk + w_cell);
  MatchBatchDev& m = c->ch_match;
  m = MatchBatchDev{};
  m.pyr_base = c->pyr.base; m.slot_bytes = c->pyr.slot_bytes; m.width = c->pyr.w[0]; m.height = c->pyr.h[0];
  m.fx = pr->cam.fx; m.fy = pr->cam.fy; m.cx = pr->cam.cx; m.cy = pr->cam.cy; m.cam_width = pr->cam.width; m.cam_height = pr->cam.height;
  m.n = (int)NC; m.n_pyr_levels = pr->n_pyr_levels; m.align_max_iter = pr->align_max_iter;
  m.frame_T = b.frame_T; m.frame_slot = b.frame_slot; m.cur_frame = r.frame; m.ref_frame = reinterpret_cast<const int*>(B + o_fref);
  m.ref_px = reinterpret_cast<const double*>(B + o_rpx); m.ref_f = reinterpret_cast<const double*>(B + o_rf); m.ref_level = reinterpret_cast<const int*>(B + o_rlevel);
  m.ref_type = B + o_rtype; m.ref_grad = reinterpret_cast<const double*>(B + o_rgrad); m.pos = b.pos; m.px_cur = r.px;
  m.px_out = reinterpret_cast<double*>(Wk + w_mpx); m.found = Wk + w_found; m.search_level = reinterpret_cast<int*>(Wk + w_slevel); m.n_iter = reinterpret_cast<int*>(Wk + w_niter);
  m.active = b.active;
  PoseBatchDev& q = c->ch_pose;
  q = PoseBatchDev{};
  q.jobs = b.po_jobs; q.state = c->ch_d_state.as<PoseStateDev>();
  q.pt_f = b.pt_f; q.pt_pos = b.pt_pos; q.pt_level = b.pt_level; q.seg_line = b.seg_line; q.seg_spos = b.seg_spos; q.seg_epos = b.seg_epos; q.seg_level = b.seg_level;
  q.pt_keep = c->ch_d_ptkeep.as<uint8_t>(); q.seg_keep = c->ch_d_segkeep.as<uint8_t>();
  q.scratch_f32 = c->ch_d_s32.as<float>(); q.scratch_f64 = c->ch_d_s64.as<double>();
  q.log = nullptr; q.log_cap = 0; q.n_jobs = n;
  c->ch_jobs.swap(jobs);
  c->ch_n = n; c->ch_ncand = (int)NC; c->ch_npt_cap = npt_total; c->ch_nseg_cap = nseg_total;
  c->ch_staged = true; c->ch_run_seq = 0;
  return PLSVO_OK;
}

extern "C" int plsvo_chain_run(plsvo_ctx* c) {
  CTX_CHECK(c);
  RoctxRange range("frame_step");
  if (!c->ch_staged || !c->a_staged || c->a_n != c->ch_n) return fail(c, PLSVO_E_STATE, "chain_run: no staged frame step (or the alignment batch was re-staged since)");
  int rc = plsvo_align_run(c); if (rc) return rc;
  HIP_TRY(c, launch_chain_pose(c->ch_b, c->stream));
  { EventPair ep{}; prof_begin(c, PLSVO_K_MATCH, &ep);
    HIP_TRY(c, launch_reproject(c->ch_reproj, c->stream));
    HIP_TRY(c, launch_chain_active(c->ch_b, c->stream));
    HIP_TRY(c, launch_match_direct(c->ch_match, c->stream));
    HIP_TRY(c, launch_chain_select(c->ch_b, c->stream));
    prof_end(c, PLSVO_K_MATCH, &ep); }
  const int cus = c->cu_count > 0 ? c->cu_count : 256;
  int threads = c->ch_n <= 2 * cus ? 256 : ((long)c->ch_b.n_cand <= 580l * c->ch_n ? 16 : 64);
  if (c->env_poseopt_threads) threads = c->env_poseopt_threads;
  c->p_refill_frames = 0;
  EventPair ep{}; prof_begin(c, PLSVO_K_POSEOPT, &ep);
  HIP_TRY(c, launch_pose_opt(c->ch_pose, c->ch_d_poses.as<double>(), threads, c->stream));
  prof_end(c, PLSVO_K_POSEOPT, &ep);
  c->ch_run_seq = ++c->run_seq;
  return PLSVO_OK;
}

extern "C" const double* plsvo_chain_poses_dev(plsvo_ctx* c) { return (c && c->ch_staged) ? c->ch_d_poses.as<double>() : nullptr; }

extern "C" int plsvo_chain_fetch(plsvo_ctx* c, int n, plsvo_chain_out* out) {
  CTX_CHECK(c);
  if (!c->ch_staged) return fail(c, PLSVO_E_STATE, "chain_fetch: no staged frame step");
  if (n != c->ch_n || !out) return fail(c, PLSVO_E_INVALID, "chain_fetch: n does not match the staged batch");
  std::vector<plsvo_align_out> ao((size_t)n);
  for (int j = 0; j < n; ++j) ao[(size_t)j].seg_alive_out = out[j].align.seg_alive_out;
  int rc = plsvo_align_fetch(c, n, ao.data()); if (rc) return rc;
  const size_t NC = (size_t)c->ch_ncand, NP = (size_t)c->ch_npt_cap, NS = (size_t)c->ch_nseg_cap;
  std::vector<PoseStateDev> st((size_t)n);
  std::vector<uint8_t> found(std::max(NC, (size_t)1)), pk(std::max(NP, (size_t)1)), sk(std::max(NS, (size_t)1));
  std::vector<double> mpx(std::max(NC * 2, (size_t)1));
  std::vector<int> slev(std::max(NC, (size_t)1)), selp(std::max(NP, (size_t)1)), sels(std::max(NS, (size_t)1)), nsel((size_t)n * 2);
  const ChainBatchDev& b = c->ch_b;
  HIP_TRY(c, hipMemcpyAsync(st.data(), c->ch_d_state.p, (size_t)n * sizeof(PoseStateDev), hipMemcpyDeviceToHost, c->stream));
  HIP_TRY(c, hipMemcpyAsync(nsel.data(), b.n_sel, (size_t)n * 2 * sizeof(int), hipMemcpyDeviceToHost, c->stream));
  if (NC) {
    HIP_TRY(c, hipMemcpyAsync(found.data(), b.found, NC, hipMemcpyDeviceToHost, c->stream));
    HIP_TRY(c, hipMemcpyAsync(mpx.data(), b.m_px, NC * 2 * sizeof(double), hipMemcpyDeviceToHost, c->stream));
    HIP_TRY(c, hipMemcpyAsync(slev.data(), b.search_level, NC * sizeof(int), hipMemcpyDeviceToHost, c->stream));
  }
  if (NP) {
    HIP_TRY(c, hipMemcpyAsync(pk.data(), c->ch_d_ptkeep.p, NP, hipMemcpyDeviceToHost, c->stream));
    HIP_TRY(c, hipMemcpyAsync(selp.data(), b.sel_pt, NP * sizeof(int), hipMemcpyDeviceToHost, c->stream));
  }
  if (NS) {
    HIP_TRY(c, hipMemcpyAsync(sk.data(), c->ch_d_segkeep.p, NS, hipMemcpyDeviceToHost, c->stream));
    HIP_TRY(c, hipMemcpyAsync(sels.data(), b.sel_seg, NS * sizeof(int), hipMemcpyDeviceToHost, c->stream));
  }
  HIP_TRY(c, hipStreamSynchronize(c->stream));
  for (int j = 0; j < n; ++j) {
    const ChainJobDev& J = c->ch_jobs[(size_t)j];
    const PoseStateDev& s = st[(size_t)j];
    plsvo_chain_out& o = out[j];
    o.align = ao[(size_t)j];
    uint8_t* pko = o.pose.pt_keep; uint8_t* sko = o.pose.seg_keep;
    memset(&o.pose, 0, sizeof(o.pose));
    o.pose.pt_keep = pko; o.pose.seg_keep = sko;
    for (int k = 0; k < 7; ++k) o.pose.T_f_w[k] = s.T[k];
    for (int k = 0; k < 36; ++k) o.pose.cov[k] = s.cov[k];
    o.pose.estimated_scale = s.estimated_scale; o.pose.error_init = s.error_init; o.pose.error_final = s.error_final;
    o.pose.num_obs_pt = s.num_obs_pt; o.pose.num_obs_ls = s.num_obs_ls;
    o.pose.iters = s.iters; o.pose.iters_ref = s.iters_ref; o.pose.status = s.status;
    o.n_sel_pt = nsel[(size_t)j * 2]; o.n_sel_seg = nsel[(size_t)j * 2 + 1];
    const int nc = J.n_pt + 2 * J.n_seg;
    if (pko && o.n_sel_pt > 0) memcpy(pko, pk.data() + J.po_pt_off, (size_t)o.n_sel_pt);
    if (sko && o.n_sel_seg > 0) memcpy(sko, sk.data() + J.po_seg_off, (size_t)o.n_sel_seg);
    if (o.found && nc) memcpy(o.found, found.data() + J.cand_off, (size_t)nc);
    if (o.px && nc) memcpy(o.px, mpx.data() + 2 * (size_t)J.cand_off, (size_t)nc * 2 * sizeof(double));
    if (o.search_level && nc) memcpy(o.search_level, slev.data() + J.cand_off, (size_t)nc * sizeof(int));
    if (o.sel_pt && o.n_sel_pt > 0) memcpy(o.sel_pt, selp.data() + J.po_pt_off, (size_t)o.n_sel_pt * sizeof(int));
    if (o.sel_seg && o.n_sel_seg > 0) memcpy(o.sel_seg, sels.data() + J.po_seg_off, (size_t)o.n_sel_seg * sizeof(int));
  }
  return PLSVO_OK;
}

extern "C" int plsvo_frame_step_batch(plsvo_ctx* c, int n, const plsvo_chain_in* in, const plsvo_chain_params* params, plsvo_chain_out* out) {
  int rc = plsvo_chain_stage(c, n, in, params); if (rc) return rc;
  rc = plsvo_chain_run(c); if (rc) return rc;
  return plsvo_chain_fetch(c, n, out);
}

extern "C" int plsvo_trajectory_record(const double T_f_w[7], const double cov[36], double out7[7]) {
  if (!T_f_w || !cov || !out7) return 0;
  bool skip_frame = false;
  for (int i = 0; i < 36; ++i) if (!((1.e-16 < std::fabs(cov[i])) && (std::fabs(cov[i]) < 1.e+16))) skip_frame = true;
  const SE3d W = se3_inv(se3_load(T_f_w));
  if ((W.t[0] == 0. && W.t[1] == 0. && W.t[2] == 0.) && (W.q.x == -0. && W.q.y == -0. && W.q.z == -0. && W.q.w == 1.)) skip_frame = true;
  out7[0] = W.t[0]; out7[1] = W.t[1]; out7[2] = W.t[2]; out7[3] = W.q.x; out7[4] = W.q.y; out7[5] = W.q.z; out7[6] = W.q.w;
  return skip_frame ? 0 : 1;
}

extern "C" int plsvo_update_seeds(plsvo_ctx* c, const plsvo_seeds_in* in, plsvo_seeds_out* out) {
  CTX_CHECK(c);
  if (!in || !out || in->n_pt < 0 || in->n_seg < 0 || in->n_frames < 0 || in->n_pyr_levels < 1 || in->align_max_iter < 0 || in->max_epi_search_steps < 0)
    return fail(c, PLSVO_E_INVALID, "update_seeds: bad arguments");
  const int np = in->n_pt, ns = in->n_seg, nf = in->n_frames;
// ... 174 lines not shown
```

pl-svo_amd/csrc/poseopt_kernels.hip:

```cpp
#include <hip/hip_runtime.h>

#include "plsvo_dev.hpp"
#include "plsvo_math.hpp"
#include "plsvo_wave.hpp"
#include "poseopt_refill.hpp"

#ifndef PLSVO_POSEOPT_WAVES
#define PLSVO_POSEOPT_WAVES 3
#endif
#ifdef PLSVO_WAVE_EMU
#define PLSVO_PO_OCC(T)
#else
#define PLSVO_PO_OCC(T) __attribute__((amdgpu_waves_per_eu((T) == 64 ? PLSVO_POSEOPT_WAVES : 1, (T) == 64 ? PLSVO_POSEOPT_WAVES : 8)))
#endif
#if defined(PLSVO_POSEOPT_ROWS_WAVES) && !defined(PLSVO_WAVE_EMU)
#define PLSVO_PO_ROWS_OCC __attribute__((amdgpu_waves_per_eu(PLSVO_POSEOPT_ROWS_WAVES, PLSVO_POSEOPT_ROWS_WAVES)))
#else
#define PLSVO_PO_ROWS_OCC
#endif
namespace plsvo_hip {

#ifdef PLSVO_TIMING
#define PTICK(slot) do { if (threadIdx.x == 0) { const unsigned long long t__ = __builtin_amdgcn_s_memtime(); s_time[slot] += t__ - s_tlast; s_tlast = t__; } } while (0)
#else
#define PTICK(slot) do { } while (0)
#endif

#define PO_RED 32
#ifndef PO_RADIX_BITS
#define PO_RADIX_BITS 8
#endif
#define PO_BINS (1 << PO_RADIX_BITS)

template <int PO_T, int BITS, typename U, typename GET>
__device__ U block_radix_select(GET get, int n, int k, int* s_hist, int* s_sel) {
  const int tid = threadIdx.x, lane = tid & 63, wave = tid >> 6;
  U prefix = 0, mask = 0;
  int shift = BITS;
  while (shift > 0) {
    const int bits = shift >= PO_RADIX_BITS ? PO_RADIX_BITS : shift;
    shift -= bits;
    const int nb = 1 << bits;
    for (int i = tid; i < PO_BINS; i += PO_T) s_hist[i] = 0;
    __syncthreads();
    for (int i = tid; i < n; i += PO_T) {
      const U v = get(i);
      if ((v & mask) == prefix) atomicAdd(&s_hist[(int)((v >> shift) & (U)(nb - 1))], 1);
    }
    __syncthreads();
    constexpr int PER = PO_BINS >= PO_T ? PO_BINS / PO_T : 1;
    const bool owner = tid * PER < PO_BINS;
    int loc[PER]; int local = 0;
#pragma unroll
    for (int j = 0; j < PER; ++j) { loc[j] = owner ? s_hist[tid * PER + j] : 0; local += loc[j]; }
    int incl = local;
#pragma unroll
    for (int d = 1; d < 64; d <<= 1) { const int v = __shfl_up(incl, d, 64); if (lane >= d) incl += v; }
    if (lane == 63) s_sel[4 + wave] = incl;
    __syncthreads();
    int wave_off = 0;
    for (int w = 0; w < wave; ++w) wave_off += s_sel[4 + w];
    int cum = wave_off + incl - local;
#pragma unroll
    for (int j = 0; j < PER; ++j) {
      if (owner && k >= cum && k < cum + loc[j]) { s_sel[0] = tid * PER + j; s_sel[1] = k - cum; s_sel[2] = loc[j]; }
      cum += loc[j];
    }
    __syncthreads();
    prefix |= ((U)s_sel[0]) << shift;
    mask |= ((U)(nb - 1)) << shift;
    k = s_sel[1];
    const int survivors = s_sel[2];
    __syncthreads();
    if (survivors == 1 && shift > 0) {
      for (int i = tid; i < n; i += PO_T) {
        const U v = get(i);
        if ((v & mask) == prefix) { s_hist[0] = (int)(unsigned)(v & (U)0xffffffffu); s_hist[1] = (int)(unsigned)((unsigned long long)v >> 32); }
      }
      __syncthreads();
      const U r = (U)(((unsigned long long)(unsigned)s_hist[1] << 32) | (unsigned long long)(unsigned)s_hist[0]);
      __syncthreads();
      return r;
    }
  }
  return prefix;
}


// ... 349 lines not shown
    { const unsigned long long t__ = __builtin_amdgcn_s_memtime(); s_time[4] += t__ - s_tlast; }
    for (int k = 0; k < 8; ++k) st->phase_ticks[k] = s_time[k];
#endif
  }
}

#define DPP_ROW_SHR_(n) (0x110 + (n))
template <int N>
__device__ __forceinline__ int row_shr_i32(int v) { return __builtin_amdgcn_update_dpp(0, v, DPP_ROW_SHR_(N), 0xf, 0xf, true); }
__device__ __forceinline__ int row_scan_incl_i32(int v) {
  v += row_shr_i32<1>(v); v += row_shr_i32<2>(v); v += row_shr_i32<4>(v); v += row_shr_i32<8>(v);
  return v;
}
__device__ __forceinline__ int row_sum_i32(int v) {
  v += __builtin_amdgcn_update_dpp(0, v, DPP_QUAD_XOR1, 0xf, 0xf, true);
  v += __builtin_amdgcn_update_dpp(0, v, DPP_QUAD_XOR2, 0xf, 0xf, true);
  v += __builtin_amdgcn_update_dpp(0, v, DPP_ROW_HALF_MIRROR, 0xf, 0xf, true);
  v += __builtin_amdgcn_update_dpp(0, v, DPP_ROW_MIRROR, 0xf, 0xf, true);
  return v;
}

struct PoseRowLds {
  double pose[32];
  double tot[32];
  double lu[36];
  double x[8];
  int perm[8];
  int ctl[8];
  int sel[8];
  int hist[PO_BINS];
};

template <int BITS, typename U, typename GET>
__device__ __forceinline__ U row_radix_select(GET get, int n, int k, bool active, int* hist, int* sel) {
  static_assert(PO_RADIX_BITS == 8 && BITS % 8 == 0, "16 lanes x 16 bins");
  const int rl = threadIdx.x & 15;
  U prefix = 0, mask = 0, result = 0;
  bool done = !active;
  for (int shift = BITS - 8; shift >= 0; shift -= 8) {
    if (!__any(!done)) break;
#pragma unroll
    for (int j = 0; j < 16; j += 4) *reinterpret_cast<uint4*>(hist + rl * 16 + j) = make_uint4(0u, 0u, 0u, 0u);
    wave_lds_fence();
    if (!done) for (int i = rl; i < n; i += 16) {
      const U v = get(i);
      if ((v & mask) == prefix) atomicAdd(&hist[(int)((v >> shift) & (U)255)], 1);
    }
    wave_lds_fence();
    int loc[16], local = 0;
#pragma unroll
    for (int j = 0; j < 16; j += 4) {
      const uint4 h4 = *reinterpret_cast<const uint4*>(hist + rl * 16 + j);
      loc[j] = (int)h4.x; loc[j + 1] = (int)h4.y; loc[j + 2] = (int)h4.z; loc[j + 3] = (int)h4.w;
    }
#pragma unroll
    for (int j = 0; j < 16; ++j) local += loc[j];
    int cum = row_scan_incl_i32(local) - local;
    if (!done) {
#pragma unroll
      for (int j = 0; j < 16; ++j) {
        if (k >= cum && k < cum + loc[j]) { sel[0] = rl * 16 + j; sel[1] = k - cum; sel[2] = loc[j]; }
        cum += loc[j];
      }
    }
    wave_lds_fence();
    bool single = false;
    if (!done) {
      prefix |= ((U)(unsigned)sel[0]) << shift;
      mask |= ((U)255) << shift;
      k = sel[1];
      single = sel[2] == 1 && shift > 0;
      if (single) for (int i = rl; i < n; i += 16) {
        const U v = get(i);
        if ((v & mask) == prefix) { sel[4] = (int)(unsigned)(v & (U)0xffffffffu); sel[5] = (int)(unsigned)((unsigned long long)v >> 32); }
      }
    }
    wave_lds_fence();
    if (single) { result = (U)(((unsigned long long)(unsigned)sel[5] << 32) | (unsigned long long)(unsigned)sel[4]); done = true; }
    wave_lds_fence();
  }
  return done ? result : prefix;
}

__device__ __forceinline__ void lane_solve6(const double* tot, double* xs, double* x, int flavour) {
  double key[6]; int idx[6];
#pragma unroll
  for (int i = 0; i < 6; ++i) { key[i] = fabs(tot[sym6_index(i, i)]); idx[i] = i; }
#pragma unroll
  for (int k = 0; k < 5; ++k) {
    double bk = key[k]; int bi = idx[k], bp = k;
#pragma unroll
    for (int j = k + 1; j < 6; ++j) {
      const bool better = key[j] > bk || (bk != bk && key[j] == key[j]);
      if (better) { bk = key[j]; bi = idx[j]; bp = j; }
    }
    const double ok_ = key[k]; const int oi = idx[k];
#pragma unroll
    for (int j = k + 1; j < 6; ++j) if (bp == j) { key[j] = ok_; idx[j] = oi; }
    key[k] = bk; idx[k] = bi;
  }
  double M[6][6], r[6];
#pragma unroll
  for (int a = 0; a < 6; ++a) {
#pragma unroll
    for (int c = 0; c < 6; ++c) M[a][c] = tot[sym6_index(idx[a], idx[c])];
    r[a] = tot[21 + idx[a]];
  }
  unsigned zero_piv = 0u;
  const double cutoff = flavour == 330 ? 0.0 : fabs(2.220446049250313e-16 * key[0]);
#pragma unroll
  for (int p = 0; p < 6; ++p) {
    const double piv = M[p][p];
    if (!(key[p] < cutoff) && fabs(piv) > cutoff) {
      const double rinv = fast_rcp(piv);
#pragma unroll
      for (int i = 0; i < 6; ++i) {
        if (i == p) continue;
        const double f = M[i][p];
#pragma unroll
        for (int j = p + 1; j < 6; ++j) M[i][j] = fma(-(f * M[p][j]), rinv, M[i][j]);
        r[i] = fma(-(f * r[p]), rinv, r[i]);
      }
    } else {
      zero_piv |= 1u << p;
    }
  }
  const double tolerance = 1.0 / 1.7976931348623157e308;
#pragma unroll
  for (int a = 0; a < 6; ++a) {
    const double dgi = M[a][a], m = r[a];
    double xi = (((zero_piv >> a) & 1u) || !(fabs(dgi) > tolerance)) ? ((dgi != dgi || m != m) ? (m + dgi) : 0.0) : m / dgi;
    if (cutoff > 1.7976931348623157e308) xi = (a == 5 || fabs(dgi) <= 1.7976931348623157e308) ? 0.0 : __builtin_nan("");
    xs[idx[a]] = xi;
  }
  __builtin_amdgcn_fence(__ATOMIC_RELEASE, "workgroup"); __builtin_amdgcn_fence(__ATOMIC_ACQUIRE, "workgroup");
#pragma unroll
  for (int c = 0; c < 6; ++c) x[c] = xs[c];
}

__device__ __forceinline__ void rows_gn_loop(const PoseBatchDev& b, const PoseJobDev& job, PoseStateDev* st, int job_id, PoseRowLds& L, bool row_on,
                                             int n_iter, int phase, double scale_pt, double scale_ls, double* init_vec, const double* obs) {
  const int lane = threadIdx.x & 63, rl = lane & 15;
  const int nf = job.n_pts + job.n_seg;
  bool running = row_on && n_iter > 0;
  for (int iter = 0; __any(running); ++iter) {
    double acc[32];
#pragma unroll
    for (int k = 0; k < 32; ++k) acc[k] = 0.0;
    if (running) {
      double P[12];
#pragma unroll
      for (int k = 0; k < 12; ++k) P[k] = L.pose[k];
      for (int f = rl; f < nf; f += 16) popt_accumulate_feature(b, job, f, P, scale_pt, scale_ls, iter == 0, init_vec, obs, acc);
    }
    double out2[2];
    row_reduce_scatter32(acc, out2);
    if (running) *reinterpret_cast<double2*>(L.tot + row_reduce_scatter32_index(lane)) = make_double2(out2[0], out2[1]);
    wave_lds_fence();
    if (running && rl == 0) {
      double dT[6];
      lane_solve6(L.tot, L.x, dT, job.ldlt_flavour);
      const double new_chi2 = L.tot[27];
      L.pose[27] += L.tot[28]; L.pose[28] += L.tot[29];
      L.ctl[1 + phase] += 1;
      SE3d model = se3_load(L.pose + 12);
      int accepted = 1, brk = 0;
      if ((iter > 0 && new_chi2 > L.pose[26]) || isnan(dT[0])) {
        model = se3_load(L.pose + 19); accepted = 0; brk = 1;
      } else {
        const SE3d Tn = se3_mul_dev(se3_exp_dev(dT), model);
        se3_store(model, L.pose + 19);
        model = Tn; L.pose[26] = new_chi2;
        if (norm_max6(dT) <= 0.0000000001) brk = 1;
      }
      if (iter + 1 >= n_iter) brk = 1;
      se3_store(model, L.pose + 12);
      quat_to_matrix(model.q, L.pose); L.pose[9] = model.t[0]; L.pose[10] = model.t[1]; L.pose[11] = model.t[2];
      L.ctl[0] = brk;
      if (b.log) {
        const int lc = st->log_count;
        if (lc < b.log_cap) {
          plsvo_poseopt_iterlog* r = b.log + (size_t)job_id * b.log_cap + lc;
          r->phase = phase; r->iter = iter; r->accepted = accepted; r->reserved0 = 0; r->new_chi2 = new_chi2;
          for (int k = 0; k < 6; ++k) r->dT[k] = dT[k];
          se3_store(model, r->T_after);
          for (int i = 0; i < 6; ++i) for (int jj = 0; jj < 6; ++jj) r->A[i * 6 + jj] = L.tot[sym6_index(i, jj)];
          for (int k = 0; k < 6; ++k) r->b[k] = L.tot[21 + k];
        }
        st->log_count = lc + 1;
      }
    }
    wave_lds_fence();
    if (running && L.ctl[0]) running = false;
  }
}

__global__ __launch_bounds__(64) PLSVO_PO_ROWS_OCC void pose_opt_rows_kernel(PoseBatchDev b, double* poses) {
  __shared__ __align__(16) PoseRowLds s_rows[4];
  const int lane = threadIdx.x & 63, row = lane >> 4, rl = lane & 15;
  const int job_raw = blockIdx.x * 4 + row;
  const bool row_valid = job_raw < b.n_jobs;
  const int job_id = row_valid ? (b.order ? b.order[job_raw] : job_raw) : b.n_jobs - 1;
  const PoseJobDev job = b.jobs[job_id];
  PoseStateDev* st = b.state + job_id;
  PoseRowLds& L = s_rows[row];
  const int np = job.n_pts, ns = job.n_seg, nf = np + ns;

  const size_t fbase = (size_t)job.pt_off + (size_t)job.seg_off;
  float* errs = b.scratch_f32 + fbase;
  double* vec = b.scratch_f64 + 5 * fbase;

  if (row_valid && rl == 0) {
    SE3d m = se3_load(job.T0);
    se3_store(m, L.pose + 12); se3_store(m, L.pose + 19); L.pose[26] = 0.0; L.pose[27] = 0.0; L.pose[28] = 0.0;
    for (int k = 0; k < 32; ++k) L.tot[k] = 0.0;
    quat_to_matrix(m.q, L.pose); L.pose[9] = m.t[0]; L.pose[10] = m.t[1]; L.pose[11] = m.t[2];
    L.ctl[0] = 0; L.ctl[1] = 0; L.ctl[2] = 0;
    st->log_count = 0; st->status = 0; st->iters = 0; st->iters_ref = 0; st->pt_iters = 0; st->seg_iters = 0;
    st->num_obs_pt = 0; st->num_obs_ls = 0; st->estimated_scale = 0; st->error_init = 0; st->error_final = 0;
    for (int k = 0; k < 36; ++k) st->cov[k] = 0.0;
    for (int k = 0; k < 7; ++k) st->T[k] = job.T0[k];
    for (int k = 0; k < 8; ++k) st->phase_ticks[k] = 0;
    if (nf == 0) { st->status = 1; if (poses) for (int k = 0; k < 7; ++k) poses[7 * job_id + k] = job.T0[k]; }
    if (b.work_key) b.work_key[job_id] = 0;
  }
  const bool row_on = row_valid && nf > 0;
  if (row_on) {
    for (int i = rl; i < np; i += 16) b.pt_keep[job.pt_off + i] = 1;
    for (int s = rl; s < ns; s += 16) b.seg_keep[job.seg_off + s] = 1;
  }
  wave_lds_fence();

  if (row_on) {
    double P[12];
#pragma unroll
    for (int k = 0; k < 12; ++k) P[k] = L.pose[k];
    for (int f = rl; f < nf; f += 16) errs[f] = popt_scale_error(b, job, f, P, vec + 3 * nf);
  }
  wave_lds_fence();
  double scale_pt = 1.0, scale_ls = 1.0;
  {
    const uint32_t m_pt = row_radix_select<32, uint32_t>([&](int i) { return (uint32_t)__float_as_uint(errs[i]); }, np, np / 2, row_on && np > 0, L.hist, L.sel);
    const uint32_t m_ls = row_radix_select<32, uint32_t>([&](int i) { return (uint32_t)__float_as_uint(errs[np + i]); }, ns, ns / 2, row_on && ns > 0, L.hist, L.sel);
    if (np > 0) scale_pt = (double)__fmul_rn(1.48f, __uint_as_float(m_pt));
    if (ns > 0) scale_ls = (double)__fmul_rn(1.48f, __uint_as_float(m_ls));
  }

  if (row_on && job.n_iter <= 0) for (int f = rl; f < nf; f += 16) vec[f] = __longlong_as_double(0x7ff0000000000000LL);
  rows_gn_loop(b, job, st, job_id, L, row_on, job.n_iter, 0, scale_pt, scale_ls, vec, vec + 3 * nf);

  if (row_on) {
    const double f2 = job.fx * job.fx;
    for (int t = rl; t < 36; t += 16) L.lu[t] = L.tot[sym6_index(t / 6, t % 6)] * f2;
  }
  wave_lds_fence();
  if (row_on && rl == 0) lu6_lds(L.lu, L.perm);
  wave_lds_fence();
  if (row_on && rl < 6) inv6_column_lds(L.lu, L.perm, rl, st->cov);

  const double thr_pt = job.reproj_thresh / job.fx;
  const double thr_ls = thr_pt * scale_ls / scale_pt;
  int del_pt = 0, del_ls = 0;
  if (row_on) {
    double P[12];
#pragma unroll
    for (int k = 0; k < 12; ++k) P[k] = L.pose[k];
    for (int f = rl; f < nf; f += 16) {
      int deleted;
      vec[2 * nf + f] = popt_cull_feature(b, job, f, P, thr_pt, thr_ls, vec + 3 * nf, deleted);
      del_pt += deleted == 1; del_ls += deleted == 2;
      vec[nf + f] = __longlong_as_double(0x7ff0000000000000LL);
    }
  }
  const int n_del_pt = row_sum_i32(del_pt), n_del_ls = row_sum_i32(del_ls);
  wave_lds_fence();

  int n_init = job.n_iter > 0 ? nf : 0;
  rows_gn_loop(b, job, st, job_id, L, row_on && job.n_iter_ref >= 0, job.n_iter_ref, 1, scale_pt, scale_ls, vec + nf, vec + 3 * nf);
  if (job.n_iter_ref > 0) n_init += nf - n_del_pt - n_del_ls;
  wave_lds_fence();

  const unsigned long long mi = row_radix_select<64, unsigned long long>([&](int i) { return (unsigned long long)__double_as_longlong(vec[i]); },
                                                                         (job.n_iter_ref > 0) ? 2 * nf : nf, n_init / 2, row_on && n_init > 0, L.hist, L.sel);
  const unsigned long long mf = row_radix_select<64, unsigned long long>([&](int i) { return (unsigned long long)__double_as_longlong(vec[2 * nf + i]); },
                                                                         nf, nf / 2, row_on, L.hist, L.sel);
  if (row_on && rl == 0) {
    for (int k = 0; k < 7; ++k) st->T[k] = L.pose[12 + k];
    if (poses) for (int k = 0; k < 7; ++k) poses[7 * job_id + k] = L.pose[12 + k];
    st->error_init = n_init > 0 ? sqrt(__longlong_as_double((long long)mi)) * job.fx : 0.0;
    st->error_final = sqrt(__longlong_as_double((long long)mf)) * job.fx;
    st->estimated_scale = scale_pt * job.fx;
    st->num_obs_pt = (unsigned long long)(np - n_del_pt);
    st->num_obs_ls = (unsigned long long)(ns - n_del_ls);
    st->iters = L.ctl[1]; st->iters_ref = L.ctl[2];
    st->pt_iters = (unsigned long long)(L.pose[27] + 0.5); st->seg_iters = (unsigned long long)(L.pose[28] + 0.5);
    if (b.work_key) b.work_key[job_id] = (int)fmin(L.pose[27] + L.pose[28] + 0.5, 2147483647.0);
  }
}

#ifdef PLSVO_WAVE_EMU
__device__ __forceinline__ void quat_to_matrix_rows(const Quat& q, double* R) { quat_to_matrix(q, R); }
#else
__device__ __forceinline__ void quat_to_matrix_rows(const Quat& q, double* R) {
#pragma clang fp contract(off)
  const double tx = 2.0 * q.x, ty = 2.0 * q.y, tz = 2.0 * q.z;
  const double twx = tx * q.w, twy = ty * q.w, twz = tz * q.w;
  const double tyy = ty * q.y, tzz = tz * q.z;
  R[0] = 1.0 - fma(q.y, ty, tzz); R[1] = fma(q.x, ty, -twz);      R[2] = fma(q.x, tz, twy);
  R[3] = fma(q.x, ty, twz);       R[4] = 1.0 - fma(q.x, tx, tzz); R[5] = fma(q.y, tz, -twx);
  R[6] = fma(q.x, tz, -twy);      R[7] = fma(q.y, tz, twx);       R[8] = 1.0 - fma(q.x, tx, tyy);
}
#endif

__global__ __launch_bounds__(64) PLSVO_PO_ROWS_OCC void pose_refill_prologue_kernel(PoseBatchDev b, PoseRefillDev q, double* poses) {
  __shared__ __align__(16) PoseRowLds s_rows[4];
  const int lane = threadIdx.x & 63, row = lane >> 4, rl = lane & 15;
  const int job_raw = blockIdx.x * 4 + row;
  const bool row_valid = job_raw < b.n_jobs;
  const int job_id = row_valid ? job_raw : b.n_jobs - 1;
  const PoseJobDev job = b.jobs[job_id];
  PoseStateDev* st = b.state + job_id;
  PoseRowLds& L = s_rows[row];
  const int np = job.n_pts, ns = job.n_seg, nf = np + ns;
  const size_t fbase = (size_t)job.pt_off + (size_t)job.seg_off;
  float* errs = b.scratch_f32 + fbase;
  double* vec = b.scratch_f64 + 5 * fbase;

  if (row_valid && rl == 0) {
    SE3d m = se3_load(job.T0);
    se3_store(m, L.pose + 12); se3_store(m, L.pose + 19); L.pose[26] = 0.0; L.pose[27] = 0.0; L.pose[28] = 0.0;
    L.pose[29] = 0.0; L.pose[30] = 0.0; L.pose[31] = 0.0;
    quat_to_matrix_rows(m.q, L.pose); L.pose[9] = m.t[0]; L.pose[10] = m.t[1]; L.pose[11] = m.t[2];
    st->log_count = 0; st->status = 0; st->iters = 0; st->iters_ref = 0; st->pt_iters = 0; st->seg_iters = 0;
    st->num_obs_pt = 0; st->num_obs_ls = 0; st->estimated_scale = 0; st->error_init = 0; st->error_final = 0;
    for (int k = 0; k < 36; ++k) st->cov[k] = 0.0;
    for (int k = 0; k < 7; ++k) st->T[k] = job.T0[k];
    for (int k = 0; k < 8; ++k) st->phase_ticks[k] = 0;
    if (nf == 0) { st->status = 1; if (poses) for (int k = 0; k < 7; ++k) poses[7 * job_id + k] = job.T0[k]; }
    if (b.work_key) b.work_key[job_id] = 0;
  }
  const bool row_on = row_valid && nf > 0;
  if (row_on) {
    for (int i = rl; i < np; i += 16) b.pt_keep[job.pt_off + i] = 1;
    for (int s = rl; s < ns; s += 16) b.seg_keep[job.seg_off + s] = 1;
  }
  wave_lds_fence();

  if (row_on) {
    double P[12];
#pragma unroll
    for (int k = 0; k < 12; ++k) P[k] = L.pose[k];
    for (int f = rl; f < nf; f += 16) errs[f] = popt_scale_error(b, job, f, P, vec + 3 * nf);
  }
  wave_lds_fence();
  double scale_pt = 1.0, scale_ls = 1.0;
  {
    const uint32_t m_pt = row_radix_select<32, uint32_t>([&](int i) { return (uint32_t)__float_as_uint(errs[i]); }, np, np / 2, row_on && np > 0, L.hist, L.sel);
    const uint32_t m_ls = row_radix_select<32, uint32_t>([&](int i) { return (uint32_t)__float_as_uint(errs[np + i]); }, ns, ns / 2, row_on && ns > 0, L.hist, L.sel);
    if (np > 0) scale_pt = (double)__fmul_rn(1.48f, __uint_as_float(m_pt));
    if (ns > 0) scale_ls = (double)__fmul_rn(1.48f, __uint_as_float(m_ls));
  }
  if (row_on && job.n_iter <= 0) for (int f = rl; f < nf; f += 16) vec[f] = __longlong_as_double(0x7ff0000000000000LL);

  if (row_valid) {
    PoseRefillCarry& c = q.carry[job_id];
    *reinterpret_cast<double2*>(c.pose + 2 * rl) = *reinterpret_cast<const double2*>(L.pose + 2 * rl);
    *reinterpret_cast<double2*>(c.tot + 2 * rl) = make_double2(0.0, 0.0);
    if (rl == 0) { c.scale_pt = scale_pt; c.scale_ls = scale_ls; c.iters = 0; }
  }
}

__global__ __launch_bounds__(64) PLSVO_PO_ROWS_OCC void pose_refill_gn_kernel(PoseBatchDev b, PoseRefillDev q) {
  __shared__ __align__(16) PoseRowLds s_rows[4];
  const int lane = threadIdx.x & 63, row = lane >> 4, rl = lane & 15;
  PoseRowLds& L = s_rows[row];
  PoseJobDev job;
  job.n_pts = 0; job.n_seg = 0; job.pt_off = 0; job.seg_off = 0; job.n_iter = 0; job.ldlt_flavour = 320;
  int job_id = 0, nf = 0, iter = 0;
  double scale_pt = 1.0, scale_ls = 1.0;
  double* vec = b.scratch_f64;
  bool running = false, want = true;
  for (;;) {
    while (__any(want)) {
      if (want && rl == 0) L.sel[6] = atomicAdd(q.next, 1);
      wave_lds_fence();
      if (want) {
        const int slot = L.sel[6];
        if (slot >= b.n_jobs) {
          want = false;
        } else {
          job_id = b.order ? b.order[slot] : slot;
          const PoseJobDev* J = b.jobs + job_id;
          job.n_pts = J->n_pts; job.n_seg = J->n_seg; job.pt_off = J->pt_off; job.seg_off = J->seg_off; job.n_iter = J->n_iter; job.ldlt_flavour = J->ldlt_flavour;
          nf = job.n_pts + job.n_seg;
          if (nf > 0 && job.n_iter > 0) {
            const PoseRefillCarry& c = q.carry[job_id];
            *reinterpret_cast<double2*>(L.pose + 2 * rl) = *reinterpret_cast<const double2*>(c.pose + 2 * rl);
            if (rl == 0) { L.ctl[0] = 0; L.ctl[1] = 0; }
            scale_pt = c.scale_pt; scale_ls = c.scale_ls;
            vec = b.scratch_f64 + 5 * ((size_t)job.pt_off + (size_t)job.seg_off);
            iter = 0; running = true; want = false;
          }
        }
      }
      wave_lds_fence();
    }
    if (!__any(running)) break;

    double acc[32];
#pragma unroll
    for (int k = 0; k < 32; ++k) acc[k] = 0.0;
    if (running) {
      double P[12];
#pragma unroll
      for (int k = 0; k < 12; ++k) P[k] = L.pose[k];
      for (int f = rl; f < nf; f += 16) popt_accumulate_feature(b, job, f, P, scale_pt, scale_ls, iter == 0, vec, vec + 3 * nf, acc);
    }
    double out2[2];
    row_reduce_scatter32(acc, out2);
    if (running) *reinterpret_cast<double2*>(L.tot + row_reduce_scatter32_index(lane)) = make_double2(out2[0], out2[1]);
    wave_lds_fence();
    if (running && rl == 0) {
      double dT[6];
      lane_solve6(L.tot, L.x, dT, job.ldlt_flavour);
      const double new_chi2 = L.tot[27];
      L.pose[27] += L.tot[28]; L.pose[28] += L.tot[29];
      L.ctl[1] += 1;
      SE3d model = se3_load(L.pose + 12);
      int brk = 0;
      if ((iter > 0 && new_chi2 > L.pose[26]) || isnan(dT[0])) {
        model = se3_load(L.pose + 19); brk = 1;
      } else {
        const SE3d Tn = se3_mul_dev(se3_exp_dev(dT), model);
        se3_store(model, L.pose + 19);
        model = Tn; L.pose[26] = new_chi2;
        if (norm_max6(dT) <= 0.0000000001) brk = 1;
      }
      if (iter + 1 >= job.n_iter) brk = 1;
      se3_store(model, L.pose + 12);
      quat_to_matrix_rows(model.q, L.pose); L.pose[9] = model.t[0]; L.pose[10] = model.t[1]; L.pose[11] = model.t[2];
      L.ctl[0] = brk;
    }
    wave_lds_fence();
    if (running) {
      ++iter;
      if (L.ctl[0]) {
        PoseRefillCarry& c = q.carry[job_id];
        *reinterpret_cast<double2*>(c.pose + 2 * rl) = *reinterpret_cast<const double2*>(L.pose + 2 * rl);
        *reinterpret_cast<double2*>(c.tot + 2 * rl) = *reinterpret_cast<const double2*>(L.tot + 2 * rl);
        if (rl == 0) c.iters = L.ctl[1];
        running = false; want = true;
      }
    }
  }
}

__global__ __launch_bounds__(64) PLSVO_PO_ROWS_OCC void pose_refill_epilogue_kernel(PoseBatchDev b, PoseRefillDev q, double* poses) {
  __shared__ __align__(16) PoseRowLds s_rows[4];
  const int lane = threadIdx.x & 63, row = lane >> 4, rl = lane & 15;
  const int job_raw = blockIdx.x * 4 + row;
  const bool row_valid = job_raw < b.n_jobs;
  const int job_id = row_valid ? job_raw : b.n_jobs - 1;
  const PoseJobDev job = b.jobs[job_id];
  PoseStateDev* st = b.state + job_id;
  PoseRowLds& L = s_rows[row];
  const int np = job.n_pts, ns = job.n_seg, nf = np + ns;
  const size_t fbase = (size_t)job.pt_off + (size_t)job.seg_off;
  double* vec = b.scratch_f64 + 5 * fbase;
  const bool row_on = row_valid && nf > 0;
  const PoseRefillCarry& c = q.carry[job_id];
  *reinterpret_cast<double2*>(L.pose + 2 * rl) = *reinterpret_cast<const double2*>(c.pose + 2 * rl);
  *reinterpret_cast<double2*>(L.tot + 2 * rl) = *reinterpret_cast<const double2*>(c.tot + 2 * rl);
  const double scale_pt = c.scale_pt, scale_ls = c.scale_ls;
  const int iters = c.iters;
  wave_lds_fence();

  if (row_on) {
    const double f2 = job.fx * job.fx;
    for (int t = rl; t < 36; t += 16) L.lu[t] = L.tot[sym6_index(t / 6, t % 6)] * f2;
  }
  wave_lds_fence();
  if (row_on && rl == 0) lu6_lds(L.lu, L.perm);
  wave_lds_fence();
  if (row_on && rl < 6) inv6_column_lds(L.lu, L.perm, rl, st->cov);

  const double thr_pt = job.reproj_thresh / job.fx;
  const double thr_ls = thr_pt * scale_ls / scale_pt;
  int del_pt = 0, del_ls = 0;
  if (row_on) {
    double P[12];
#pragma unroll
    for (int k = 0; k < 12; ++k) P[k] = L.pose[k];
    for (int f = rl; f < nf; f += 16) {
      int deleted;
      vec[2 * nf + f] = popt_cull_feature(b, job, f, P, thr_pt, thr_ls, vec + 3 * nf, deleted);
      del_pt += deleted == 1; del_ls += deleted == 2;
      vec[nf + f] = __longlong_as_double(0x7ff0000000000000LL);
    }
  }
  const int n_del_pt = row_sum_i32(del_pt), n_del_ls = row_sum_i32(del_ls);
  wave_lds_fence();

  const int n_init = job.n_iter > 0 ? nf : 0;
  const unsigned long long mi = row_radix_select<64, unsigned long long>([&](int i) { return (unsigned long long)__double_as_longlong(vec[i]); },
                                                                         nf, n_init / 2, row_on && n_init > 0, L.hist, L.sel);
  const unsigned long long mf = row_radix_select<64, unsigned long long>([&](int i) { return (unsigned long long)__double_as_longlong(vec[2 * nf + i]); },
                                                                         nf, nf / 2, row_on, L.hist, L.sel);
  if (row_on && rl == 0) {
    for (int k = 0; k < 7; ++k) st->T[k] = L.pose[12 + k];
    if (poses) for (int k = 0; k < 7; ++k) poses[7 * job_id + k] = L.pose[12 + k];
    st->error_init = n_init > 0 ? sqrt(__longlong_as_double((long long)mi)) * job.fx : 0.0;
    st->error_final = sqrt(__longlong_as_double((long long)mf)) * job.fx;
    st->estimated_scale = scale_pt * job.fx;
    st->num_obs_pt = (unsigned long long)(np - n_del_pt);
    st->num_obs_ls = (unsigned long long)(ns - n_del_ls);
    st->iters = iters; st->iters_ref = 0;
    st->pt_iters = (unsigned long long)(L.pose[27] + 0.5); st->seg_iters = (unsigned long long)(L.pose[28] + 0.5);
    if (b.work_key) b.work_key[job_id] = (int)fmin(L.pose[27] + L.pose[28] + 0.5, 2147483647.0);
  }
}

bool pose_opt_refill_built() {
#ifdef PLSVO_TIMING
  return false;
#else
  return true;
#endif
}

hipError_t launch_pose_opt_refill(const PoseBatchDev& b, const PoseRefillDev& q, double* d_poses, int gn_grid, hipStream_t stream) {
  const int wgs = (b.n_jobs + 3) / 4;
  if (gn_grid < 1 || gn_grid > wgs) return hipErrorInvalidValue;
  hipLaunchKernelGGL(pose_refill_prologue_kernel, dim3(wgs), dim3(64), 0, stream, b, q, d_poses);
  hipLaunchKernelGGL(pose_refill_gn_kernel, dim3(gn_grid), dim3(64), 0, stream, b, q);
  hipLaunchKernelGGL(pose_refill_epilogue_kernel, dim3(wgs), dim3(64), 0, stream, b, q, d_poses);
  return hipGetLastError();
}

hipError_t launch_pose_opt(const PoseBatchDev& b, double* d_poses, int threads, hipStream_t stream) {
  switch (threads) {
    case 16: hipLaunchKernelGGL(pose_opt_rows_kernel, dim3((b.n_jobs + 3) / 4), dim3(64), 0, stream, b, d_poses); break;
    case 64: hipLaunchKernelGGL((pose_opt_kernel<64>), dim3(b.n_jobs), dim3(64), 0, stream, b, d_poses); break;
    case 256: hipLaunchKernelGGL((pose_opt_kernel<256>), dim3(b.n_jobs), dim3(256), 0, stream, b, d_poses); break;
    case 512: hipLaunchKernelGGL((pose_opt_kernel<512>), dim3(b.n_jobs), dim3(512), 0, stream, b, d_poses); break;
    default: return hipErrorInvalidValue;
  }
  return hipGetLastError();
}

}
```

pl-svo_amd/csrc/poseopt_refill.hpp:

```cpp
#pragma once
#include <hip/hip_runtime.h>

#include "plsvo_dev.hpp"

namespace plsvo_hip {

struct PoseRefillCarry {
  double pose[32];
  double tot[32];
  double scale_pt, scale_ls;
  int iters;
  int reserved[3];
};

struct PoseRefillDev {
  PoseRefillCarry* carry;
  int* next;
};

bool pose_opt_refill_built();
hipError_t launch_pose_opt_refill(const PoseBatchDev& b, const PoseRefillDev& q, double* d_poses, int gn_grid, hipStream_t stream);

}
```

Baseline: 2.300 million.

## Replace row radix median select with register-held values and rank finish

Replaces the per-row 64/32-bit radix select used for robust-scale and error medians in the pose optimiser kernels with a new select. It loads values into registers (up to 320 per row) and narrows the starting digit using a DPP min/max over the row, so it skips the leading digits the values share. It finishes by ranking once few candidates remain, falling back to the old path above capacity. It is on by default behind a new option and adds a standalone test kernel and API, at the cost of extra register pressure in the row kernels.

```diff
diff --git a/include/plsvo_hip.h b/include/plsvo_hip.h
--- a/include/plsvo_hip.h
+++ b/include/plsvo_hip.h
@@ -38,6 +38,7 @@
 #define PLSVO_OPT_POSEOPT_REORDER 5
 #define PLSVO_OPT_ALIGN_TAIL_SPLIT 6
 #define PLSVO_OPT_POSEOPT_REFILL 7
+#define PLSVO_OPT_POSEOPT_SELECT 8
 int plsvo_hip_set_option(plsvo_ctx* ctx, int option, int value);
 const char* plsvo_hip_last_error(const plsvo_ctx* ctx);
 void* plsvo_hip_stream(plsvo_ctx* ctx);
@@ -208,6 +209,23 @@
 int plsvo_poseopt_copy_poses(plsvo_ctx* ctx, double* d_dst);
 int plsvo_poseopt_work(plsvo_ctx* ctx, uint64_t* pt_iters, uint64_t* seg_iters);
 int plsvo_poseopt_refill_frames(plsvo_ctx* ctx, int* refill_frames);
+#define PLSVO_ROW_SELECT_CAP 320
+#define PLSVO_ROW_SELECT_EQUAL 1
+#define PLSVO_ROW_SELECT_RANK 2
+#define PLSVO_ROW_SELECT_EXTRA_PASS 4
+#define PLSVO_ROW_SELECT_FALLBACK 8
+#define PLSVO_ROW_SELECT_DIGITS 16
+typedef struct {
+  int32_t bits;
+  int32_t n_rows;
+  const void* patterns;
+  int64_t n_patterns;
+  const int64_t* row_off;
+  const int32_t* row_n;
+  const int32_t* row_k;
+  const uint8_t* row_active;
+} plsvo_row_select_in;
+int plsvo_poseopt_row_select(plsvo_ctx* ctx, const plsvo_row_select_in* in, void* selected, int32_t* path);
 
 
 typedef struct plsvo_structopt_in {
diff --git a/pl-svo_amd/abi.py b/pl-svo_amd/abi.py
--- a/pl-svo_amd/abi.py
+++ b/pl-svo_amd/abi.py
@@ -115,6 +115,11 @@
 
 class MatchWarpOut(C.Structure):
     _fields_ = [("A", c_double_p), ("search_level", c_i32_p), ("warped", c_u8_p), ("patch", c_u8_p), ("staged", c_u8_p)]
+
+
+class RowSelectIn(C.Structure):
+    _fields_ = [("bits", C.c_int32), ("n_rows", C.c_int32), ("patterns", C.c_void_p), ("n_patterns", C.c_int64),
+                ("row_off", C.POINTER(C.c_int64)), ("row_n", c_i32_p), ("row_k", c_i32_p), ("row_active", c_u8_p)]
 
 
 class ReprojectIn(C.Structure):
diff --git a/pl-svo_amd/capi.py b/pl-svo_amd/capi.py
--- a/pl-svo_amd/capi.py
+++ b/pl-svo_amd/capi.py
@@ -18,7 +18,7 @@
     "plsvo_sparse_align", "plsvo_sparse_align_batch", "plsvo_align_stage", "plsvo_align_run", "plsvo_align_fetch",
     "plsvo_align_set_trace", "plsvo_align_fetch_trace", "plsvo_align_poses_dev", "plsvo_align_copy_poses", "plsvo_align_work", "plsvo_align_work_points", "plsvo_align_chi2_ties", "plsvo_align_launch_order", "plsvo_align_tail_frames",
     "plsvo_pose_optimize", "plsvo_pose_optimize_batch", "plsvo_poseopt_stage", "plsvo_poseopt_run", "plsvo_poseopt_fetch",
-    "plsvo_poseopt_set_trace", "plsvo_poseopt_fetch_trace", "plsvo_poseopt_poses_dev", "plsvo_poseopt_copy_poses", "plsvo_poseopt_work", "plsvo_poseopt_refill_frames",
+    "plsvo_poseopt_set_trace", "plsvo_poseopt_fetch_trace", "plsvo_poseopt_poses_dev", "plsvo_poseopt_copy_poses", "plsvo_poseopt_work", "plsvo_poseopt_refill_frames", "plsvo_poseopt_row_select",
     "plsvo_structure_optimize", "plsvo_match_direct", "plsvo_match_warp_patches", "plsvo_reproject", "plsvo_trajectory_record", "plsvo_update_seeds",
     "plsvo_chain_stage", "plsvo_chain_run", "plsvo_chain_fetch", "plsvo_frame_step_batch", "plsvo_chain_poses_dev",
     "plsvo_pack_pose_records", "plsvo_fetch_pose_records", "plsvo_gather_poses",
@@ -112,6 +112,7 @@
         "plsvo_align_launch_order": (C.c_int, [ctxp, C.c_int, C.POINTER(C.c_int32)]),
         "plsvo_align_tail_frames": (C.c_int, [ctxp, C.POINTER(C.c_int)]),
         "plsvo_poseopt_refill_frames": (C.c_int, [ctxp, C.POINTER(C.c_int)]),
+        "plsvo_poseopt_row_select": (C.c_int, [ctxp, C.POINTER(abi.RowSelectIn), vp, abi.c_i32_p]),
         "plsvo_pose_optimize": (C.c_int, [ctxp, C.POINTER(abi.PoseOptIn), C.POINTER(abi.PoseOptOut)]),
         "plsvo_pose_optimize_batch": (C.c_int, [ctxp, C.c_int, C.POINTER(abi.PoseOptIn), C.POINTER(abi.PoseOptOut)]),
         "plsvo_poseopt_stage": (C.c_int, [ctxp, C.c_int, C.POINTER(abi.PoseOptIn)]),
@@ -189,6 +190,9 @@
     def set_poseopt_refill(self, on):
         self._chk(self.L.plsvo_hip_set_option(self.h, 7, 1 if on else 0))
 
+    def set_poseopt_select(self, on):
+        self._chk(self.L.plsvo_hip_set_option(self.h, 8, 1 if on else 0))
+
     def close(self):
         if getattr(self, "h", None):
             self.L.plsvo_hip_destroy(self.h)
@@ -358,6 +362,22 @@
         out = np.zeros(n, dtype=np.int32)
         self._chk(self.L.plsvo_align_launch_order(self.h, n, out.ctypes.data_as(C.POINTER(C.c_int32))))
         return out
+
+    def poseopt_row_select(self, patterns, row_off, row_n, row_k, row_active):
+        patterns = np.ascontiguousarray(patterns)
+        if patterns.dtype not in (np.dtype(np.uint32), np.dtype(np.uint64)):
+            raise ValueError("poseopt_row_select: patterns are uint32 or uint64")
+        off = np.ascontiguousarray(row_off, np.int64); n = np.ascontiguousarray(row_n, np.int32)
+        k = np.ascontiguousarray(row_k, np.int32); act = np.ascontiguousarray(row_active, np.uint8)
+        nr = len(n)
+        if not (len(off) == len(k) == len(act) == nr):
+            raise ValueError("poseopt_row_select: per-row arrays differ in length")
+        sel = np.zeros(nr, patterns.dtype); path = np.zeros(nr, np.int32)
+        a = abi.RowSelectIn(patterns.dtype.itemsize * 8, nr, patterns.ctypes.data_as(C.c_void_p), patterns.size,
+                            off.ctypes.data_as(C.POINTER(C.c_int64)), n.ctypes.data_as(abi.c_i32_p), k.ctypes.data_as(abi.c_i32_p),
+                            act.ctypes.data_as(abi.c_u8_p))
+        self._chk(self.L.plsvo_poseopt_row_select(self.h, C.byref(a), sel.ctypes.data_as(C.c_void_p), path.ctypes.data_as(abi.c_i32_p)))
+        return sel, path
 
     def poseopt_refill_frames(self):
         n = C.c_int(0)
diff --git a/pl-svo_amd/csrc/plsvo_capi.hip b/pl-svo_amd/csrc/plsvo_capi.hip
--- a/pl-svo_amd/csrc/plsvo_capi.hip
+++ b/pl-svo_amd/csrc/plsvo_capi.hip
@@ -15,13 +15,14 @@
 #include "plsvo_dev.hpp"
 #include "plsvo_math.hpp"
 #include "poseopt_refill.hpp"
+#include "poseopt_select.hpp"
 
 namespace plsvo_hip {
 size_t align_level_lds_bytes(int threads, int cap, int scap, int chi_lds_pts);
 hipError_t launch_align_reorder(const int* work_key, int n, int* order_out, int shift, hipStream_t stream);
 hipError_t launch_align_levels(const AlignBatchDev& b, int cap, int scap, int level_hi, int level_lo, int do_init, int threads, size_t lds,
                                hipStream_t stream);
-hipError_t launch_pose_opt(const PoseBatchDev& b, double* d_poses, int threads, hipStream_t stream);
+hipError_t launch_pose_opt(const PoseBatchDev& b, double* d_poses, int threads, int select, hipStream_t stream);
 hipError_t launch_structopt(const StructBatchDev& s, hipStream_t stream);
 hipError_t launch_match_direct(const MatchBatchDev& b, hipStream_t stream);
 hipError_t launch_match_warp_patches(const MatchBatchDev& b, hipStream_t stream);
@@ -141,6 +142,7 @@
   int env_poseopt_reorder_min = 0;
   bool opt_poseopt_refill = true;
   int env_poseopt_refill_min = 0, env_poseopt_refill_waves = 0;
+  bool opt_poseopt_select = true;
   bool p_any_ref = false;
   int p_refill_frames = 0;
   DevBuf p_d_carry, p_d_refill_next;
@@ -268,6 +270,7 @@
   c->env_poseopt_no_reorder = env_flag("PLSVO_POSEOPT_NO_REORDER");
   if (const char* s = getenv("PLSVO_POSEOPT_REORDER_MIN")) c->env_poseopt_reorder_min = atoi(s);
   if (const char* s = getenv("PLSVO_POSEOPT_REFILL")) c->opt_poseopt_refill = atoi(s) != 0;
+  if (const char* s = getenv("PLSVO_POSEOPT_SELECT")) c->opt_poseopt_select = atoi(s) != 0;
   if (const char* s = getenv("PLSVO_POSEOPT_REFILL_MIN")) c->env_poseopt_refill_min = atoi(s);
   if (const char* s = getenv("PLSVO_POSEOPT_REFILL_WAVES")) c->env_poseopt_refill_waves = atoi(s);
   c->env_host_timing = getenv("PLSVO_HOST_TIMING") != nullptr;
@@ -333,6 +336,11 @@
   if (option == PLSVO_OPT_POSEOPT_REFILL) {
     if (value != 0 && value != 1) return fail(c, PLSVO_E_INVALID, "set_option: the pose optimiser's row refill is 0 (four frames of a wave in lock step) or 1 (rows take their next frame from a queue)");
     c->opt_poseopt_refill = value != 0;
+    return PLSVO_OK;
+  }
+  if (option == PLSVO_OPT_POSEOPT_SELECT) {
+    if (value != 0 && value != 1) return fail(c, PLSVO_E_INVALID, "set_option: the row kernels' median select is 0 (radix select over memory, every digit) or 1 (values in registers, rank finish)");
+    c->opt_poseopt_select = value != 0;
     return PLSVO_OK;
   }
   return fail(c, PLSVO_E_INVALID, "set_option: unknown option");
@@ -1444,10 +1452,10 @@
     HIP_TRY(c, c->p_d_refill_next.ensure(16));
     HIP_TRY(c, hipMemsetAsync(c->p_d_refill_next.p, 0, 16, c->stream));
     const PoseRefillDev q{ c->p_d_carry.as<PoseRefillCarry>(), c->p_d_refill_next.as<int>() };
-    HIP_TRY(c, launch_pose_opt_refill(c->p_b, q, c->p_d_poses.as<double>(), gn_grid, c->stream));
+    HIP_TRY(c, launch_pose_opt_refill(c->p_b, q, c->p_d_poses.as<double>(), gn_grid, c->opt_poseopt_select ? 1 : 0, c->stream));
     c->p_refill_frames = c->p_n;
   } else {
-    HIP_TRY(c, launch_pose_opt(c->p_b, c->p_d_poses.as<double>(), threads, c->stream));
+    HIP_TRY(c, launch_pose_opt(c->p_b, c->p_d_poses.as<double>(), threads, c->opt_poseopt_select ? 1 : 0, c->stream));
   }
   c->p_run_seq = ++c->run_seq;
   prof_end(c, PLSVO_K_POSEOPT, &ep);
@@ -1495,6 +1503,50 @@
   CTX_CHECK(c);
   if (!refill_frames) return fail(c, PLSVO_E_INVALID, "poseopt_refill_frames: NULL output");
   *refill_frames = c->p_refill_frames;
+  return PLSVO_OK;
+}
+
+extern "C" int plsvo_poseopt_row_select(plsvo_ctx* c, const plsvo_row_select_in* in, void* selected, int32_t* path) {
+  CTX_CHECK(c);
+  if (!in || !selected || !path || in->n_rows < 0 || in->n_patterns < 0 || (in->bits != 32 && in->bits != 64))
+    return fail(c, PLSVO_E_INVALID, "poseopt_row_select: bad arguments");
+  const int nr = in->n_rows;
+  if (nr == 0) return PLSVO_OK;
+  if (!in->row_off || !in->row_n || !in->row_k || !in->row_active || (in->n_patterns > 0 && !in->patterns))
+    return fail(c, PLSVO_E_INVALID, "poseopt_row_select: null input array");
+  for (int r = 0; r < nr; ++r) {
+    const long long o = in->row_off[r]; const int n = in->row_n[r];
+    if (n < 0 || o < 0 || o + (long long)n > in->n_patterns) return fail(c, PLSVO_E_INVALID, "poseopt_row_select: a row lies outside the patterns");
+    if (in->row_active[r] && n > 0 && (in->row_k[r] < 0 || in->row_k[r] >= n)) return fail(c, PLSVO_E_INVALID, "poseopt_row_select: k outside [0, n)");
+  }
+  HIP_TRY(c, hipSetDevice(c->device));
+  const size_t width = (size_t)in->bits / 8;
+  auto up16 = [](size_t v) { return (v + 15) / 16 * 16; };
+  const size_t o_off = up16((size_t)in->n_patterns * width), o_n = o_off + up16((size_t)nr * sizeof(long long)), o_k = o_n + up16((size_t)nr * sizeof(int));
+  const size_t o_act = o_k + up16((size_t)nr * sizeof(int)), in_bytes = o_act + up16((size_t)nr);
+  std::vector<uint8_t> h(in_bytes, 0);
+  if (in->n_patterns > 0) memcpy(h.data(), in->patterns, (size_t)in->n_patterns * width);
+  memcpy(h.data() + o_off, in->row_off, (size_t)nr * sizeof(long long));
+  memcpy(h.data() + o_n, in->row_n, (size_t)nr * sizeof(int));
+  memcpy(h.data() + o_k, in->row_k, (size_t)nr * sizeof(int));
+  memcpy(h.data() + o_act, in->row_active, (size_t)nr);
+  const size_t o_path = up16((size_t)nr * width), out_bytes = o_path + (size_t)nr * sizeof(int);
+  HIP_TRY(c, c->s_d_in.ensure(in_bytes + 16));
+  HIP_TRY(c, c->s_d_out.ensure(out_bytes + 16));
+  char* din = reinterpret_cast<char*>(c->s_d_in.p); char* dout = reinterpret_cast<char*>(c->s_d_out.p);
+  HIP_TRY(c, hipMemcpyAsync(din, h.data(), in_bytes, hipMemcpyHostToDevice, c->stream));
+  HIP_TRY(c, hipMemsetAsync(dout, 0, out_bytes, c->stream));
+  RowSelectDev t{};
+  t.patterns = din; t.row_off = reinterpret_cast<const long long*>(din + o_off); t.row_n = reinterpret_cast<const int*>(din + o_n);
+  t.row_k = reinterpret_cast<const int*>(din + o_k); t.row_active = reinterpret_cast<const uint8_t*>(din + o_act);
+  t.selected = dout; t.path = reinterpret_cast<int*>(dout + o_path);
+  t.n_rows = nr; t.bits = in->bits; t.select = c->opt_poseopt_select ? 1 : 0;
+  HIP_TRY(c, launch_pose_row_select(t, c->stream));
+  std::vector<uint8_t> ho(out_bytes);
+  HIP_TRY(c, hipMemcpyAsync(ho.data(), dout, out_bytes, hipMemcpyDeviceToHost, c->stream));
+  HIP_TRY(c, hipStreamSynchronize(c->stream));
+  memcpy(selected, ho.data(), (size_t)nr * width);
+  memcpy(path, ho.data() + o_path, (size_t)nr * sizeof(int));
   return PLSVO_OK;
 }
 
@@ -1912,7 +1964,7 @@
   if (c->env_poseopt_threads) threads = c->env_poseopt_threads;
   c->p_refill_frames = 0;
   EventPair ep{}; prof_begin(c, PLSVO_K_POSEOPT, &ep);
-  HIP_TRY(c, launch_pose_opt(c->ch_pose, c->ch_d_poses.as<double>(), threads, c->stream));
+  HIP_TRY(c, launch_pose_opt(c->ch_pose, c->ch_d_poses.as<double>(), threads, c->opt_poseopt_select ? 1 : 0, c->stream));
   prof_end(c, PLSVO_K_POSEOPT, &ep);
   c->ch_run_seq = ++c->run_seq;
   return PLSVO_OK;
diff --git a/pl-svo_amd/csrc/poseopt_kernels.hip b/pl-svo_amd/csrc/poseopt_kernels.hip
--- a/pl-svo_amd/csrc/poseopt_kernels.hip
+++ b/pl-svo_amd/csrc/poseopt_kernels.hip
@@ -4,6 +4,7 @@
 #include "plsvo_math.hpp"
 #include "plsvo_wave.hpp"
 #include "poseopt_refill.hpp"
+#include "poseopt_select.hpp"
 
 #ifndef PLSVO_POSEOPT_WAVES
 #define PLSVO_POSEOPT_WAVES 3
@@ -519,6 +520,126 @@
   return done ? result : prefix;
 }
 
+template <int CTRL>
+__device__ __forceinline__ uint32_t dpp_mov_bits(uint32_t v) { return (uint32_t)__builtin_amdgcn_update_dpp(0, (int)v, CTRL, 0xf, 0xf, true); }
+template <int CTRL>
+__device__ __forceinline__ unsigned long long dpp_mov_bits(unsigned long long v) {
+  const uint32_t lo = dpp_mov_bits<CTRL>((uint32_t)v), hi = dpp_mov_bits<CTRL>((uint32_t)(v >> 32));
+  return ((unsigned long long)hi << 32) | (unsigned long long)lo;
+}
+template <typename U>
+__device__ __forceinline__ void row_min_max_bits(U& mn, U& mx) {
+  U a, c;
+  a = dpp_mov_bits<DPP_QUAD_XOR1>(mn); c = dpp_mov_bits<DPP_QUAD_XOR1>(mx); mn = a < mn ? a : mn; mx = c > mx ? c : mx;
+  a = dpp_mov_bits<DPP_QUAD_XOR2>(mn); c = dpp_mov_bits<DPP_QUAD_XOR2>(mx); mn = a < mn ? a : mn; mx = c > mx ? c : mx;
+  a = dpp_mov_bits<DPP_ROW_HALF_MIRROR>(mn); c = dpp_mov_bits<DPP_ROW_HALF_MIRROR>(mx); mn = a < mn ? a : mn; mx = c > mx ? c : mx;
+  a = dpp_mov_bits<DPP_ROW_MIRROR>(mn); c = dpp_mov_bits<DPP_ROW_MIRROR>(mx); mn = a < mn ? a : mn; mx = c > mx ? c : mx;
+}
+template <typename U>
+__device__ __forceinline__ U row_or_bits(U v) {
+  v |= dpp_mov_bits<DPP_QUAD_XOR1>(v); v |= dpp_mov_bits<DPP_QUAD_XOR2>(v);
+  v |= dpp_mov_bits<DPP_ROW_HALF_MIRROR>(v); v |= dpp_mov_bits<DPP_ROW_MIRROR>(v);
+  return v;
+}
+__device__ __forceinline__ uint32_t po_bits(float x) { return (uint32_t)__float_as_uint(x); }
+__device__ __forceinline__ unsigned long long po_bits(double x) { return (unsigned long long)__double_as_longlong(x); }
+__device__ __forceinline__ uint32_t po_bits(uint32_t x) { return x; }
+__device__ __forceinline__ unsigned long long po_bits(unsigned long long x) { return x; }
+
+template <int BITS, typename U>
+__device__ __forceinline__ U row_select_regs(const U (&v)[kRowSelectChunks], int n, int k, bool active, int* hist, int& path) {
+  static_assert(PO_RADIX_BITS == 8 && kRowSelectCap < 1024, "16 lanes x 16 bins; bin, count and rank share one word");
+  const int rl = threadIdx.x & 15;
+  constexpr U ONES = ~(U)0;
+  U mn = ONES, mx = 0;
+#pragma unroll
+  for (int c = 0; c < kRowSelectChunks; ++c) if (rl + 16 * c < n) { mn = v[c] < mn ? v[c] : mn; mx = v[c] > mx ? v[c] : mx; }
+  row_min_max_bits(mn, mx);
+  U result = 0;
+  bool done = !active;
+  path = 0;
+  if (active && mn == mx) { result = mn; done = true; path = kRowSelectEqual; }
+  const U diff = mn ^ mx;
+  const int hb = diff ? 63 - __builtin_clzll((unsigned long long)diff) : 0;
+  U mask = hb + 1 >= BITS ? (U)0 : (U)(ONES << (hb + 1));
+  U prefix = mn & mask;
+  int shift = hb >= 7 ? hb - 7 : 0;
+  int passes = 0, cnt = 0;
+  while (__any(!done)) {
+#pragma unroll
+    for (int j = 0; j < 16; j += 4) *reinterpret_cast<uint4*>(hist + rl * 16 + j) = make_uint4(0u, 0u, 0u, 0u);
+    wave_lds_fence();
+    if (!done) {
+#pragma unroll
+      for (int c = 0; c < kRowSelectChunks; ++c)
+        if (rl + 16 * c < n && (v[c] & mask) == prefix) atomicAdd(&hist[(int)(((v[c] & ~mask) >> shift) & (U)255)], 1);
+    }
+    wave_lds_fence();
+    int loc[16], local = 0;
+#pragma unroll
+    for (int j = 0; j < 16; j += 4) {
+      const uint4 h4 = *reinterpret_cast<const uint4*>(hist + rl * 16 + j);
+      loc[j] = (int)h4.x; loc[j + 1] = (int)h4.y; loc[j + 2] = (int)h4.z; loc[j + 3] = (int)h4.w;
+    }
+#pragma unroll
+    for (int j = 0; j < 16; ++j) local += loc[j];
+    int cum = row_scan_incl_i32(local) - local;
+    int pack = 0;
+#pragma unroll
+    for (int j = 0; j < 16; ++j) {
+      if (!done && k >= cum && k < cum + loc[j]) pack = ((rl * 16 + j) << 20) | (loc[j] << 10) | (k - cum);
+      cum += loc[j];
+    }
+    pack = row_sum_i32(pack);
+    bool rank = false;
+    if (!done) {
+      ++passes;
+      prefix |= (U)(unsigned)(pack >> 20) << shift;
+      mask |= (U)255 << shift;
+      cnt = (pack >> 10) & 1023; k = pack & 1023;
+      if (shift == 0) { result = prefix; done = true; path = kRowSelectDigits | (passes > 1 ? kRowSelectExtraPass : 0); }
+      else if (cnt <= 16) rank = true;
+      else shift = shift >= 8 ? shift - 8 : 0;
+    }
+    if (__any(rank)) {
+      U* const cand = reinterpret_cast<U*>(hist);
+      int mine = 0;
+#pragma unroll
+      for (int c = 0; c < kRowSelectChunks; ++c) mine += (rank && rl + 16 * c < n && (v[c] & mask) == prefix) ? 1 : 0;
+      int off = row_scan_incl_i32(mine) - mine;
+      if (rank) {
+#pragma unroll
+        for (int c = 0; c < kRowSelectChunks; ++c) if (rl + 16 * c < n && (v[c] & mask) == prefix) cand[off++] = v[c];
+      }
+      wave_lds_fence();
+      const bool holds = rank && rl < cnt;
+      const U me = holds ? cand[rl] : ONES;
+      int less = 0, leq = 0;
+      if (rank) {
+#pragma unroll
+        for (int j = 0; j < 16; ++j) if (j < cnt) { const U o = cand[j]; less += o < me ? 1 : 0; leq += o <= me ? 1 : 0; }
+      }
+      const U r = row_or_bits((holds && less <= k && k < leq) ? me : (U)0);
+      if (rank) { result = r; done = true; path = kRowSelectRank | (passes > 1 ? kRowSelectExtraPass : 0); }
+      wave_lds_fence();
+    }
+  }
+  return result;
+}
+
+template <int BITS, typename U, typename T>
+__device__ __forceinline__ U row_select(const T* p, int n, int k, bool active, bool use_regs, int* hist, int* sel, int& path) {
+  if (use_regs && !__any(active && n > kRowSelectCap)) {
+    const int rl = threadIdx.x & 15;
+    U v[kRowSelectChunks];
+#pragma unroll
+    for (int c = 0; c < kRowSelectChunks; ++c) { v[c] = ~(U)0; if (active && rl + 16 * c < n) v[c] = po_bits(p[rl + 16 * c]); }
+    return row_select_regs<BITS, U>(v, n, k, active, hist, path);
+  }
+  path = active ? kRowSelectFallback : 0;
+  return row_radix_select<BITS, U>([&](int i) { return (U)po_bits(p[i]); }, n, k, active, hist, sel);
+}
+
 __device__ __forceinline__ void lane_solve6(const double* tot, double* xs, double* x, int flavour) {
   double key[6]; int idx[6];
 #pragma unroll
@@ -632,7 +753,7 @@
   }
 }
 
-__global__ __launch_bounds__(64) PLSVO_PO_ROWS_OCC void pose_opt_rows_kernel(PoseBatchDev b, double* poses) {
+__global__ __launch_bounds__(64) PLSVO_PO_ROWS_OCC void pose_opt_rows_kernel(PoseBatchDev b, double* poses, int select) {
   __shared__ __align__(16) PoseRowLds s_rows[4];
   const int lane = threadIdx.x & 63, row = lane >> 4, rl = lane & 15;
   const int job_raw = blockIdx.x * 4 + row;
@@ -677,8 +798,9 @@
   wave_lds_fence();
   double scale_pt = 1.0, scale_ls = 1.0;
   {
-    const uint32_t m_pt = row_radix_select<32, uint32_t>([&](int i) { return (uint32_t)__float_as_uint(errs[i]); }, np, np / 2, row_on && np > 0, L.hist, L.sel);
-    const uint32_t m_ls = row_radix_select<32, uint32_t>([&](int i) { return (uint32_t)__float_as_uint(errs[np + i]); }, ns, ns / 2, row_on && ns > 0, L.hist, L.sel);
+    int path;
+    const uint32_t m_pt = row_select<32, uint32_t>(errs, np, np / 2, row_on && np > 0, select != 0, L.hist, L.sel, path);
+    const uint32_t m_ls = row_select<32, uint32_t>(errs + np, ns, ns / 2, row_on && ns > 0, select != 0, L.hist, L.sel, path);
     if (np > 0) scale_pt = (double)__fmul_rn(1.48f, __uint_as_float(m_pt));
     if (ns > 0) scale_ls = (double)__fmul_rn(1.48f, __uint_as_float(m_ls));
   }
@@ -717,10 +839,9 @@
   if (job.n_iter_ref > 0) n_init += nf - n_del_pt - n_del_ls;
   wave_lds_fence();
 
-  const unsigned long long mi = row_radix_select<64, unsigned long long>([&](int i) { return (unsigned long long)__double_as_longlong(vec[i]); },
-                                                                         (job.n_iter_ref > 0) ? 2 * nf : nf, n_init / 2, row_on && n_init > 0, L.hist, L.sel);
-  const unsigned long long mf = row_radix_select<64, unsigned long long>([&](int i) { return (unsigned long long)__double_as_longlong(vec[2 * nf + i]); },
-                                                                         nf, nf / 2, row_on, L.hist, L.sel);
+  int path;
+  const unsigned long long mi = row_select<64, unsigned long long>(vec, (job.n_iter_ref > 0) ? 2 * nf : nf, n_init / 2, row_on && n_init > 0, select != 0, L.hist, L.sel, path);
+  const unsigned long long mf = row_select<64, unsigned long long>(vec + 2 * nf, nf, nf / 2, row_on, select != 0, L.hist, L.sel, path);
   if (row_on && rl == 0) {
     for (int k = 0; k < 7; ++k) st->T[k] = L.pose[12 + k];
     if (poses) for (int k = 0; k < 7; ++k) poses[7 * job_id + k] = L.pose[12 + k];
@@ -749,7 +870,7 @@
 }
 #endif
 
-__global__ __launch_bounds__(64) PLSVO_PO_ROWS_OCC void pose_refill_prologue_kernel(PoseBatchDev b, PoseRefillDev q, double* poses) {
+__global__ __launch_bounds__(64) PLSVO_PO_ROWS_OCC void pose_refill_prologue_kernel(PoseBatchDev b, PoseRefillDev q, double* poses, int select) {
   __shared__ __align__(16) PoseRowLds s_rows[4];
   const int lane = threadIdx.x & 63, row = lane >> 4, rl = lane & 15;
   const int job_raw = blockIdx.x * 4 + row;
@@ -792,8 +913,9 @@
   wave_lds_fence();
   double scale_pt = 1.0, scale_ls = 1.0;
   {
-    const uint32_t m_pt = row_radix_select<32, uint32_t>([&](int i) { return (uint32_t)__float_as_uint(errs[i]); }, np, np / 2, row_on && np > 0, L.hist, L.sel);
-    const uint32_t m_ls = row_radix_select<32, uint32_t>([&](int i) { return (uint32_t)__float_as_uint(errs[np + i]); }, ns, ns / 2, row_on && ns > 0, L.hist, L.sel);
+    int path;
+    const uint32_t m_pt = row_select<32, uint32_t>(errs, np, np / 2, row_on && np > 0, select != 0, L.hist, L.sel, path);
+    const uint32_t m_ls = row_select<32, uint32_t>(errs + np, ns, ns / 2, row_on && ns > 0, select != 0, L.hist, L.sel, path);
     if (np > 0) scale_pt = (double)__fmul_rn(1.48f, __uint_as_float(m_pt));
     if (ns > 0) scale_ls = (double)__fmul_rn(1.48f, __uint_as_float(m_ls));
   }
@@ -892,7 +1014,7 @@
   }
 }
 
-__global__ __launch_bounds__(64) PLSVO_PO_ROWS_OCC void pose_refill_epilogue_kernel(PoseBatchDev b, PoseRefillDev q, double* poses) {
+__global__ __launch_bounds__(64) PLSVO_PO_ROWS_OCC void pose_refill_epilogue_kernel(PoseBatchDev b, PoseRefillDev q, double* poses, int select) {
   __shared__ __align__(16) PoseRowLds s_rows[4];
   const int lane = threadIdx.x & 63, row = lane >> 4, rl = lane & 15;
   const int job_raw = blockIdx.x * 4 + row;
@@ -939,10 +1061,9 @@
   wave_lds_fence();
 
   const int n_init = job.n_iter > 0 ? nf : 0;
-  const unsigned long long mi = row_radix_select<64, unsigned long long>([&](int i) { return (unsigned long long)__double_as_longlong(vec[i]); },
-                                                                         nf, n_init / 2, row_on && n_init > 0, L.hist, L.sel);
-  const unsigned long long mf = row_radix_select<64, unsigned long long>([&](int i) { return (unsigned long long)__double_as_longlong(vec[2 * nf + i]); },
-                                                                         nf, nf / 2, row_on, L.hist, L.sel);
+  int path;
+  const unsigned long long mi = row_select<64, unsigned long long>(vec, nf, n_init / 2, row_on && n_init > 0, select != 0, L.hist, L.sel, path);
+  const unsigned long long mf = row_select<64, unsigned long long>(vec + 2 * nf, nf, nf / 2, row_on, select != 0, L.hist, L.sel, path);
   if (row_on && rl == 0) {
     for (int k = 0; k < 7; ++k) st->T[k] = L.pose[12 + k];
     if (poses) for (int k = 0; k < 7; ++k) poses[7 * job_id + k] = L.pose[12 + k];
@@ -965,18 +1086,43 @@
 #endif
 }
 
-hipError_t launch_pose_opt_refill(const PoseBatchDev& b, const PoseRefillDev& q, double* d_poses, int gn_grid, hipStream_t stream) {
+hipError_t launch_pose_opt_refill(const PoseBatchDev& b, const PoseRefillDev& q, double* d_poses, int gn_grid, int select, hipStream_t stream) {
   const int wgs = (b.n_jobs + 3) / 4;
   if (gn_grid < 1 || gn_grid > wgs) return hipErrorInvalidValue;
-  hipLaunchKernelGGL(pose_refill_prologue_kernel, dim3(wgs), dim3(64), 0, stream, b, q, d_poses);
+  hipLaunchKernelGGL(pose_refill_prologue_kernel, dim3(wgs), dim3(64), 0, stream, b, q, d_poses, select);
   hipLaunchKernelGGL(pose_refill_gn_kernel, dim3(gn_grid), dim3(64), 0, stream, b, q);
-  hipLaunchKernelGGL(pose_refill_epilogue_kernel, dim3(wgs), dim3(64), 0, stream, b, q, d_poses);
+  hipLaunchKernelGGL(pose_refill_epilogue_kernel, dim3(wgs), dim3(64), 0, stream, b, q, d_poses, select);
   return hipGetLastError();
 }
 
-hipError_t launch_pose_opt(const PoseBatchDev& b, double* d_poses, int threads, hipStream_t stream) {
+struct RowSelectLds { int hist[PO_BINS]; int sel[8]; };
+template <int BITS, typename U>
+__global__ __launch_bounds__(64) void pose_row_select_kernel(RowSelectDev t) {
+  __shared__ __align__(16) RowSelectLds s_rows[4];
+  const int lane = threadIdx.x & 63, rl = lane & 15;
+  const int row_raw = blockIdx.x * 4 + (lane >> 4);
+  const bool valid = row_raw < t.n_rows;
+  const int row = valid ? row_raw : t.n_rows - 1;
+  const int n = t.row_n[row];
+  RowSelectLds& L = s_rows[lane >> 4];
+  int path;
+  const U r = row_select<BITS, U>(reinterpret_cast<const U*>(t.patterns) + t.row_off[row], n, t.row_k[row], valid && t.row_active[row] != 0 && n > 0,
+                                  t.select != 0, L.hist, L.sel, path);
+  if (valid && rl == 0) { reinterpret_cast<U*>(t.selected)[row] = r; t.path[row] = path; }
+}
+
+hipError_t launch_pose_row_select(const RowSelectDev& t, hipStream_t stream) {
+  if (t.n_rows < 1) return hipErrorInvalidValue;
+  const dim3 grid((t.n_rows + 3) / 4);
+  if (t.bits == 32) hipLaunchKernelGGL((pose_row_select_kernel<32, uint32_t>), grid, dim3(64), 0, stream, t);
+  else if (t.bits == 64) hipLaunchKernelGGL((pose_row_select_kernel<64, unsigned long long>), grid, dim3(64), 0, stream, t);
+  else return hipErrorInvalidValue;
+  return hipGetLastError();
+}
+
+hipError_t launch_pose_opt(const PoseBatchDev& b, double* d_poses, int threads, int select, hipStream_t stream) {
   switch (threads) {
-    case 16: hipLaunchKernelGGL(pose_opt_rows_kernel, dim3((b.n_jobs + 3) / 4), dim3(64), 0, stream, b, d_poses); break;
+    case 16: hipLaunchKernelGGL(pose_opt_rows_kernel, dim3((b.n_jobs + 3) / 4), dim3(64), 0, stream, b, d_poses, select); break;
     case 64: hipLaunchKernelGGL((pose_opt_kernel<64>), dim3(b.n_jobs), dim3(64), 0, stream, b, d_poses); break;
     case 256: hipLaunchKernelGGL((pose_opt_kernel<256>), dim3(b.n_jobs), dim3(256), 0, stream, b, d_poses); break;
     case 512: hipLaunchKernelGGL((pose_opt_kernel<512>), dim3(b.n_jobs), dim3(512), 0, stream, b, d_poses); break;
diff --git a/pl-svo_amd/csrc/poseopt_refill.hpp b/pl-svo_amd/csrc/poseopt_refill.hpp
--- a/pl-svo_amd/csrc/poseopt_refill.hpp
+++ b/pl-svo_amd/csrc/poseopt_refill.hpp
@@ -19,6 +19,6 @@
 };
 
 bool pose_opt_refill_built();
-hipError_t launch_pose_opt_refill(const PoseBatchDev& b, const PoseRefillDev& q, double* d_poses, int gn_grid, hipStream_t stream);
+hipError_t launch_pose_opt_refill(const PoseBatchDev& b, const PoseRefillDev& q, double* d_poses, int gn_grid, int select, hipStream_t stream);
 
 }
diff --git a/pl-svo_amd/csrc/poseopt_select.hpp b/pl-svo_amd/csrc/poseopt_select.hpp
--- /dev/null
+++ b/pl-svo_amd/csrc/poseopt_select.hpp
@@ -0,0 +1,28 @@
+#pragma once
+#include <hip/hip_runtime.h>
+
+#include <cstdint>
+
+namespace plsvo_hip {
+
+constexpr int kRowSelectChunks = 20;
+constexpr int kRowSelectCap = 16 * kRowSelectChunks;
+constexpr int kRowSelectEqual = 1;
+constexpr int kRowSelectRank = 2;
+constexpr int kRowSelectExtraPass = 4;
+constexpr int kRowSelectFallback = 8;
+constexpr int kRowSelectDigits = 16;
+
+struct RowSelectDev {
+  const void* patterns;
+  const long long* row_off;
+  const int* row_n;
+  const int* row_k;
+  const uint8_t* row_active;
+  void* selected;
+  int* path;
+  int n_rows, bits, select;
+};
+hipError_t launch_pose_row_select(const RowSelectDev& t, hipStream_t stream);
+
+}
```

After: 2.325 million (median of 6 runs). 1.1% higher.
